# sevagh/umx.cpp

Hardware: AMD Instinct MI355X
Metric: realtime-factor (audio-sec/wall-sec) UMX-L 4-stem, 60 s seg (higher is better)
Workload: dtype f32 (activations as 2 x fp16 planes of the power-of-two-scaled row, integer weights exact in fp16, f32 accumulate on the fp16 matrix cores; fp32-grade: 1.4-2.2x the error of an fp32 evaluation, profiles/r06_v2_accuracy_vs_float64.txt)

## Files before the change

### umx.cpp_amd/__init__.py

```python
import ctypes as C
import os
import subprocess
from pathlib import Path

import numpy as np

from . import ggml

HERE = Path(__file__).resolve().parent
ROOT = HERE.parent
NB, CROP, KX, NOUT, NFFT, HOP = 2049, 1487, 2976, 4098, 4096, 1024
SEGMENT_SAMPLES = 60 * 44100

UMX_OK, ERR_ARG, ERR_HIP, ERR_MODEL, ERR_TIMEOUT, ERR_NODEVICE = 0, 1, 2, 3, 4, 5
DTYPE_F32, DTYPE_U8, DTYPE_U16 = 0, 1, 2
FLAG_NO_WIENER = 0x1
FLAG_SOFTMASK = 0x2
FLAG_LSTM_STEPWISE = 0x10
FLAG_DEBUG_TAPS = 0x20
FLAG_LSTM_FORCE_SAFE = 0x40
FLAG_LSTM_PROFILE = 0x80
FLAG_PRECISE_ACT = 0x1000
FLAG_DEBUG_LSTM_ABORT = 0x2000
FLAG_RESIDUAL = 0x8000
# ... 383 lines not shown
        self._check(self.lib.umx_hip_weight_stems_device(self.h, (C.c_void_p * 4)(*stem_ptrs), n, hip_stream))

    def track_accumulate_device(self, track_ptrs, sum_weight_ptr, weighted_ptrs, offset, n, hip_stream=None):
        self._check(self.lib.umx_hip_track_accumulate_device(self.h, (C.c_void_p * 4)(*track_ptrs), C.c_void_p(sum_weight_ptr),
                                                             (C.c_void_p * 4)(*weighted_ptrs), offset, n, hip_stream))

    def track_normalise_device(self, track_ptrs, sum_weight_ptr, length, hip_stream=None):
        self._check(self.lib.umx_hip_track_normalise_device(self.h, (C.c_void_p * 4)(*track_ptrs), C.c_void_p(sum_weight_ptr), length,
                                                            hip_stream))

    def separate(self, wave, flags=0, shift_offset=None, rate=MODEL_RATE):
        wave = np.asarray(wave, np.float32)
        L = wave.shape[1]
        a = np.ascontiguousarray(wave.T).ravel()
        outs = [np.empty(2 * L, np.float32) for _ in range(4)]
        if rate == MODEL_RATE:
            self.separate_interleaved(a, L, outs, flags, shift_offset)
        else:
            arr = (_fp * 4)(*[o.ctypes.data_as(_fp) for o in outs])
            self._check(self.lib.umx_hip_shift_inference_rate(self.h, a.ctypes.data_as(_fp), L, int(rate),
                                                              -1 if shift_offset is None else shift_offset, arr, flags, None, None))
        return [np.ascontiguousarray(o.reshape(L, 2).T) for o in outs]

    def separate_many(self, waves, flags=0, shift_offsets=None, rates=None):
        nt = len(waves)
        ins = [np.ascontiguousarray(np.asarray(w, np.float32).T).ravel() for w in waves]
        Ls = [np.asarray(w).shape[1] for w in waves]
        outs = [[np.empty(2 * L, np.float32) for _ in range(4)] for L in Ls]
        a = (_fp * nt)(*[x.ctypes.data_as(_fp) for x in ins])
        o = (_fp * (4 * nt))(*[x.ctypes.data_as(_fp) for t4 in outs for x in t4])
        sh = (C.c_int * nt)(*[(-1 if s is None else s) for s in (shift_offsets or [None] * nt)])
        if rates is None:
            self._check(self.lib.umx_hip_separate_tracks(self.h, nt, a, (C.c_int * nt)(*Ls), sh, o, flags, None, None))
        else:
            self._check(self.lib.umx_hip_separate_tracks_rate(self.h, nt, a, (C.c_int * nt)(*Ls), (C.c_int * nt)(*rates), sh, o, flags,
                                                              None, None))
        return [[np.ascontiguousarray(x.reshape(L, 2).T) for x in t4] for t4, L in zip(outs, Ls)]

    def resample_device(self, rate_in, rate_out, in_ptrs, n_in, out_ptrs, n_out, hip_stream=None):
        nb = len(in_ptrs)
        assert len(out_ptrs) == nb
        self._check(self.lib.umx_hip_resample_device(self.h, int(rate_in), int(rate_out), nb, (C.c_void_p * nb)(*in_ptrs), int(n_in),
                                                     (C.c_void_p * nb)(*out_ptrs), int(n_out), hip_stream))

    def separate_interleaved(self, a, L, outs, flags=0, shift_offset=None):
        import time
        arr = (_fp * 4)(*[o.ctypes.data_as(_fp) for o in outs])
        t0 = time.perf_counter()
        if shift_offset is None:
            rc = self.lib.umx_hip_split_inference(self.h, a.ctypes.data_as(_fp), L, arr, flags, None, None)
        else:
            rc = self.lib.umx_hip_shift_inference(self.h, a.ctypes.data_as(_fp), L, shift_offset, arr, flags, None, None)
        dt = time.perf_counter() - t0
        self._check(rc)
        return dt

    def infer_segment(self, wave, flags=0):
        wave = np.asarray(wave, np.float32)
        n = wave.shape[1]
        a = np.ascontiguousarray(wave.T).ravel()
        outs = [np.empty(2 * n, np.float32) for _ in range(4)]
        arr = (_fp * 4)(*[o.ctypes.data_as(_fp) for o in outs])
        self._check(self.lib.umx_hip_infer_segment(self.h, a.ctypes.data_as(_fp), n, arr, flags))
        return [np.ascontiguousarray(o.reshape(n, 2).T) for o in outs]

    def infer_batch(self, waves, flags=0):
        nb = len(waves)
        aud, ns, outs = (C.c_void_p * nb)(), (C.c_int * nb)(), (C.c_void_p * (4 * nb))()
        keep = []
        for i, wv in enumerate(waves):
            if wv is None:
                aud[i], ns[i] = None, 0
                continue
            wv = np.asarray(wv, np.float32)
            a = np.ascontiguousarray(wv.T).ravel()
            o = [np.empty(2 * wv.shape[1], np.float32) for _ in range(4)]
            keep.append((a, o))
            aud[i], ns[i] = a.ctypes.data, wv.shape[1]
            for t in range(4):
                outs[4 * i + t] = o[t].ctypes.data
        self._check(self.lib.umx_hip_infer_batch(self.h, nb, aud, ns, outs, flags))
        res, k = [], 0
        for wv in waves:
            if wv is None:
                res.append(None)
                continue
            n = keep[k][0].size // 2
            res.append([np.ascontiguousarray(o.reshape(n, 2).T) for o in keep[k][1]])
            k += 1
        return res

    def infer_batch_ptrs(self, audio_ptrs, ns, out_ptrs, flags=0, where="device"):
        nb = len(audio_ptrs)
        aud = (C.c_void_p * nb)(*[p or None for p in audio_ptrs])
        n_ = (C.c_int * nb)(*ns)
        outs = (C.c_void_p * (4 * nb))(*[p or None for p in out_ptrs])
        fn = self.lib.umx_hip_infer_batch_device if where == "device" else self.lib.umx_hip_infer_batch_async
        self._check(fn(self.h, nb, aud, n_, outs, flags))

    def infer_segment_device(self, audio_ptr, n, out_ptrs, flags=0):
        arr = (C.c_void_p * 4)(*out_ptrs)
        self._check(self.lib.umx_hip_infer_segment_device(self.h, C.c_void_p(audio_ptr), n, arr, flags))

    def sync(self):
        self._check(self.lib.umx_hip_sync(self.h))

    def last_error(self):
        return self.lib.umx_hip_last_error(self.h).decode()

    def lstm_was_persistent(self):
        return bool(self.lib.umx_hip_lstm_was_persistent(self.h))

    def lstm_mode(self):
        return self.lib.umx_hip_lstm_mode(self.h)

    def lstm_profile(self):
        buf = (C.c_ulonglong * 48)()
        self._check(self.lib.umx_hip_debug_lstm_profile(self.h, buf))
        a = np.array(buf[:], dtype=np.uint64).reshape(3, 2, 8)
        return a

    def gemm_kernel_name(self, mode):
        return self.lib.umx_hip_gemm_kernel_name(self.h, mode).decode()

    def lstm_kernel_name(self):
        return self.lib.umx_hip_lstm_kernel_name(self.h).decode()

    def lstm_placement(self, n=256):
        buf = (C.c_ulonglong * n)()
        self._check(self.lib.umx_hip_debug_lstm_placement(self.h, buf, n))
        a = np.array(buf[:], dtype=np.uint64)
        return [(int(v >> 48) & 15, int(v >> 40) & 255, int(v >> 32) & 255, int(v) & 0xffffffff) for v in a]

    def tap(self, what, target=0):
        n = self.lib.umx_hip_read_tap(self.h, what.encode(), target, None, 0)
        if n < 0:
            raise UmxError(ERR_ARG, f"tap {what!r} unavailable ({n})")
        buf = np.empty(n, np.float32)
        got = self.lib.umx_hip_read_tap(self.h, what.encode(), target, buf.ctypes.data_as(_fp), n)
        if got != n:
            raise UmxError(ERR_HIP, f"tap {what!r} failed ({got})")
        T, H = self.T, self.hidden
        what = what.split("@")[0].split("#")[0]
        if what in ("lstm_l0", "lstm_l1"):
            return buf.reshape(T, H)
        if what == "proj":
            return buf.reshape(T, 4 * H)
        if what in ("spec", "y"):
            return buf.view(np.complex64).reshape(2, T, NB)
        if what in ("mix_mag", "target_mag"):
            return buf.reshape(2, T, NB)
        if what == "x":
            return buf.reshape(T, KX)
        if what in ("fc1", "lstm", "fc2"):
            return buf.reshape(T, H)
        if what == "mask":
            return buf.reshape(T, NOUT)
        return buf

    def stage_times(self, slot=None):
        names = (C.c_char_p * 32)()
        ms = (C.c_float * 32)()
        if slot is None:
            n = self.lib.umx_hip_stage_times(self.h, names, ms, 32)
        else:
            n = self.lib.umx_hip_stage_times_slot(self.h, slot, names, ms, 32)
        return {names[i].decode(): float(ms[i]) for i in range(n)}

    def stage_kernel_times(self, slot=None):
        names = (C.c_char_p * 32)()
        ms = (C.c_float * 32)()
        n = self.lib.umx_hip_stage_times_slot(self.h, 0, names, (C.c_float * 32)(), 32)
        m = self.lib.umx_hip_stage_kernel_times_slot(self.h, -1 if slot is None else slot, ms, 32)
        return {names[i].decode(): float(ms[i]) for i in range(min(n, m))}


HOST_SYMBOLS = ["umx_model_load", "umx_model_free", "umx_model_hidden", "umx_model_n_tensors", "umx_model_views",
                "umx_model_data_bytes", "umx_model_load_progress", "umx_model_dequantize", "umx_wav_load",
                "umx_wav_free", "umx_wav_write_f32", "umx_wav_load_rate", "umx_wav_write_f32_rate", "umx_split_inference", "umx_shift_inference",
                "umx_segment_plan", "umx_transition_weight", "umx_split_inference_carry", "umx_split_inference_targets"]

SEGMENT_FN = C.CFUNCTYPE(C.c_int, C.c_void_p, _fp, C.c_int, C.POINTER(_fp))
RESET_FN = C.CFUNCTYPE(C.c_int, C.c_void_p)
PROGRESS_FN = C.CFUNCTYPE(None, C.c_float, C.c_void_p)


PH_BEGIN_FN = C.CFUNCTYPE(C.c_int, C.c_void_p, _fp, C.c_int)
PH_LAYER_FN = C.CFUNCTYPE(C.c_int, C.c_void_p, C.c_int)
PH_END_FN = C.CFUNCTYPE(C.c_int, C.c_void_p, C.POINTER(_fp))
PH_STATE_FN = C.CFUNCTYPE(C.c_int, C.c_void_p, C.c_int, _fp)
P2P_FN = C.CFUNCTYPE(C.c_int, C.c_void_p, _fp, C.c_size_t, C.c_int)


class PhasedBackend(C.Structure):
    _fields_ = [("begin", PH_BEGIN_FN), ("layer", PH_LAYER_FN), ("end", PH_END_FN), ("get_layer", PH_STATE_FN),
                ("set_layer", PH_STATE_FN), ("layer_floats", C.c_size_t), ("user", C.c_void_p)]


TG_BEGIN_FN = C.CFUNCTYPE(C.c_int, C.c_void_p, _fp, C.c_int, C.c_uint)
TG_STATE_FN = C.CFUNCTYPE(C.c_int, C.c_void_p, C.c_int, C.c_int, _fp)
TG_VOID_FN = C.CFUNCTYPE(C.c_int, C.c_void_p)
TG_MAG_FN = C.CFUNCTYPE(C.c_int, C.c_void_p, C.c_int, _fp)


class TargetBackend(C.Structure):
    _fields_ = [("begin", TG_BEGIN_FN), ("layer", PH_LAYER_FN), ("get_state", TG_STATE_FN), ("set_state", TG_STATE_FN),
                ("masks", TG_VOID_FN), ("get_mag", TG_MAG_FN), ("set_mag", TG_MAG_FN), ("finish", PH_END_FN), ("discard", TG_VOID_FN),
                ("target_layer_floats", C.c_size_t), ("mag_floats", C.c_size_t), ("user", C.c_void_p)]


class P2P(C.Structure):
    _fields_ = [("send", P2P_FN), ("recv", P2P_FN), ("user", C.c_void_p)]


class Backend(C.Structure):
    _fields_ = [("segment", SEGMENT_FN), ("reset", RESET_FN), ("user", C.c_void_p)]


_host = None


def host_lib():
    global _host
    if _host is not None:
        return _host
    path = HERE / "libumx_host.so"
    if not path.exists():
        raise ImportError(f"{path} is missing: run __graft_entry__.build()")
    lib = C.CDLL(str(path))
    lib.umx_model_load.argtypes = [C.c_char_p, C.POINTER(C.c_void_p), C.c_char_p]
    lib.umx_model_free.argtypes = [C.c_void_p]
    lib.umx_model_hidden.argtypes = [C.c_void_p]
    lib.umx_model_n_tensors.argtypes = [C.c_void_p]
    lib.umx_model_views.restype = C.POINTER(TensorView)
    lib.umx_model_views.argtypes = [C.c_void_p]
    lib.umx_model_data_bytes.restype = C.c_size_t
    lib.umx_model_data_bytes.argtypes = [C.c_void_p]
    lib.umx_model_load_progress.restype = C.c_float
    lib.umx_model_load_progress.argtypes = [C.c_void_p]
    lib.umx_model_dequantize.restype = C.c_long
    lib.umx_model_dequantize.argtypes = [C.c_void_p, C.c_int, C.c_char_p, _fp, C.c_size_t]
    lib.umx_wav_load.argtypes = [C.c_char_p, C.POINTER(_fp), C.POINTER(C.c_int), C.POINTER(C.c_int), C.c_char_p]
    lib.umx_wav_free.argtypes = [_fp]
    lib.umx_wav_write_f32.argtypes = [C.c_char_p, _fp, C.c_int, C.c_char_p]
    lib.umx_wav_load_rate.argtypes = [C.c_char_p, C.POINTER(_fp), C.POINTER(C.c_int), C.POINTER(C.c_int), C.POINTER(C.c_int), C.c_char_p]
    lib.umx_wav_write_f32_rate.argtypes = [C.c_char_p, _fp, C.c_int, C.c_int, C.c_char_p]
    lib.umx_split_inference.argtypes = [C.POINTER(Backend), _fp, C.c_int, C.c_int, C.POINTER(_fp), PROGRESS_FN,
                                        C.c_void_p, C.c_char_p]
    lib.umx_shift_inference.argtypes = [C.POINTER(Backend), _fp, C.c_int, C.c_int, C.c_int, C.POINTER(_fp),
                                        PROGRESS_FN, C.c_void_p, C.c_char_p]
    lib.umx_split_inference_carry.argtypes = [C.POINTER(PhasedBackend), C.POINTER(P2P), C.c_int, C.c_int, _fp, C.c_int, C.c_int,
                                              C.POINTER(_fp), C.c_char_p]
    lib.umx_split_inference_targets.argtypes = [C.POINTER(TargetBackend), C.POINTER(P2P), C.c_int, C.c_int, _fp, C.c_int, C.c_int,
                                                C.POINTER(_fp), C.c_char_p]
    lib.umx_segment_plan.argtypes = [C.c_int, C.c_int, C.POINTER(C.c_int), C.POINTER(C.c_int), C.c_int]
    lib.umx_transition_weight.restype = C.c_float
    lib.umx_transition_weight.argtypes = [C.c_int, C.c_int, C.c_int]
    _host = lib
    return lib


class HostError(RuntimeError):
    def __init__(self, code, msg):
        super().__init__(f"umx_host error {code}: {msg}")
        self.code = code


class HostModel:

    def __init__(self, path):
        self.lib = host_lib()
        h = C.c_void_p()
        err = C.create_string_buffer(256)
        rc = self.lib.umx_model_load(str(path).encode(), C.byref(h), err)
        if rc:
            raise HostError(rc, err.value.decode())
        self.h = h
        self.hidden = self.lib.umx_model_hidden(h)
        self.n_tensors = self.lib.umx_model_n_tensors(h)

    def views(self):
        return self.lib.umx_model_views(self.h), self.n_tensors

    def dequantize(self, target, name):
        n = self.lib.umx_model_dequantize(self.h, target, name.encode(), None, 0)
        if n < 0:
            raise KeyError(name)
        a = np.empty(n, np.float32)
        self.lib.umx_model_dequantize(self.h, target, name.encode(), a.ctypes.data_as(_fp), n)
        return a

    def data_bytes(self):
        return self.lib.umx_model_data_bytes(self.h)

    def close(self):
        if getattr(self, "h", None):
            self.lib.umx_model_free(self.h)
            self.h = None

    def __del__(self):
        try:
            self.close()
        except Exception:
            pass


def engine_from_host_model(hm, segment_samples=SEGMENT_SAMPLES, device=0):
# ... 195 lines not shown
```

### umx.cpp_amd/csrc/engine.hip

```cpp
#include "../../include/umx_hip.h"
#include <chrono>
#include <dlfcn.h>

#include <algorithm>
#include <numeric>
#include <cmath>
#include <cstdio>
#include <cstdlib>
#include <cstring>
#include <map>
#include <mutex>
#include <string>
#include <vector>

#include "common.h"
#include "gemm_bf16x3.h"
#include "gemm_planes.h"
#include "gemm_planes_pp.h"
#include "gemm_planes_ps.h"
#include "lstm_kernels.h"
#include "lstm_batch.h"
#include "lstm_batch8.h"
#include "track_kernels.h"
#include "resample.h"
#include "stft_kernels.h"
#include "wiener_kernels.h"
#include "wiener_istft.h"
#include "wiener_em.h"
#include "residual_mask.h"
#include "softmask.h"
#include "gate_debug.h"

using namespace umx;

#define UMX_HIP_CHECK_CTX(ctx_, expr)                                                                                \
    do                                                                                                               \
    {                                                                                                                \
        hipError_t _e = (expr);                                                                                      \
        if (_e != hipSuccess)                                                                                        \
        {                                                                                                            \
            (ctx_)->set_error(std::string(#expr) + ": " + hipGetErrorString(_e));                                    \
            return UMX_ERR_HIP;                                                                                      \
        }                                                                                                            \
    } while (0)

namespace
{
std::string g_create_error = "";

enum { W_FC1 = 0, W_IH0, W_IH1, W_IH2, W_FC2, W_FC3, W_COUNT };
inline int gemm_weight(int mode, int layer) { return mode == G_FC1 ? W_FC1 : mode == G_IH ? W_IH0 + layer : mode == G_FC2 ? W_FC2 : W_FC3; }

struct GemmWeight
{
    const void *p = nullptr;
    int form = 0;
    float s[2] = {1.f, 1.f}, o[2] = {0.f, 0.f};
};

struct TargetBufs
{
    GemmWeight w[W_COUNT];
    float *in_scale = nullptr, *in_mean = nullptr, *bn1[4] = {};
    float *ih_b[3] = {};
    float *bn2[4] = {};
    float *bn3[4] = {}, *out_scale = nullptr, *out_mean = nullptr;
};

struct TargetAct
{
    float *cat = nullptr, *la = nullptr, *lb = nullptr, *P = nullptr, *a2 = nullptr,
          *mag = nullptr;
    unsigned short *xs_p = nullptr, *cat_p = nullptr, *la_p = nullptr, *lb_p = nullptr, *a2_p = nullptr;
    float *rs_xs = nullptr, *rs_catL = nullptr, *rs_catR = nullptr, *rs_la = nullptr, *rs_lb = nullptr, *rs_a2 = nullptr;
    float *rsc_xs = nullptr, *rsc_a2 = nullptr;
};

enum
{
    ST_STFT = 0,
    ST_FC1,
    ST_IH0,
    ST_LSTM0,
    ST_IH1,
    ST_LSTM1,
    ST_IH2,
    ST_LSTM2,
    ST_FC2,
    ST_FC3,
    ST_WIENER,
    ST_ISTFT,
    ST_OLA,
    ST_COUNT
};
enum { SP_XS = 0, SP_CATL, SP_LA, SP_LB, SP_CATR, SP_A2 };
const char *kStageNames[ST_COUNT] = {"stft",  "fc1", "lstm_ih0", "lstm_rec0", "lstm_ih1", "lstm_rec1", "lstm_ih2",
                                     "lstm_rec2", "fc2", "fc3_mask", "wiener",  "istft",    "ola"};

namespace
{
struct RoctxApi
{
    int (*push)(const char *) = nullptr;
    int (*pop)() = nullptr;
    char names[ST_COUNT][40];
    RoctxApi()
    {
        for (int i = 0; i < ST_COUNT; ++i)
            snprintf(names[i], sizeof names[i], "umx:%s", kStageNames[i]);
        const char *want = getenv("UMX_ROCTX");
        const bool force = want && atoi(want) != 0;
        for (const char *lib : {"librocprofiler-sdk-roctx.so", "libroctx64.so"})
            if (void *h = dlopen(lib, force ? (RTLD_NOW | RTLD_LOCAL) : (RTLD_NOW | RTLD_NOLOAD)))
            {
                push = reinterpret_cast<int (*)(const char *)>(dlsym(h, "roctxRangePushA"));
                pop = reinterpret_cast<int (*)()>(dlsym(h, "roctxRangePop"));
                if (push && pop)
                    return;
                push = nullptr;
                pop = nullptr;
            }
    }
};
thread_local bool t_stage_range_open = false;
inline void stage_range(int stage)
{
    static const RoctxApi api;
    if (!api.push)
        return;
    if (t_stage_range_open)
        api.pop();
    t_stage_range_open = stage >= 0 && stage < ST_COUNT;
    if (t_stage_range_open)
        api.push(api.names[stage]);
}
struct StageRangeCloser
{
    ~StageRangeCloser() { stage_range(-1); }
};
}

struct Lane
{
    TargetAct ta[4];
    float2 *spec = nullptr, *y = nullptr, *frames = nullptr;
    float *x = nullptr, *wpart = nullptr, *Rc = nullptr;
    unsigned *maxabs = nullptr;
};

struct Slot
{
    hipStream_t stream = nullptr;
    Lane lane[LSTMB_MAX_TRACKS];
    float *hbuf = nullptr;
    float *wv = nullptr;
    bool lstm_wrote_planes[3] = {false, false, false};
    bool lstm_rows_f32[3] = {true, true, true};
    unsigned *status = nullptr, *lsync = nullptr;
    unsigned long long *lprof = nullptr;
    hipEvent_t ev[ST_COUNT + 1] = {};
    hipEvent_t evk[ST_COUNT] = {};
    bool evk_set[ST_COUNT] = {};
    hipEvent_t rec_done[3] = {};
    hipEvent_t k_done = nullptr;
    hipEvent_t out_free = nullptr;
    bool out_free_valid = false;
    bool have_times = false, last_persistent = false, used = false;
};
}

namespace
{
struct LstmGate
{
    std::mutex m;
    struct Grid
    {
        hipEvent_t done;
        int units;
        hipStream_t stream;
        unsigned long long seq;
    };
    std::vector<Grid> inflight;
    std::vector<hipEvent_t> pool;
    unsigned long long seq = 0;
    int reserved = 0;
    std::vector<int> reservations;
};
LstmGate g_gate[16];

template <class Launch> hipError_t lstm_gate_launch(int device, hipStream_t st, int units, int capacity_units, Launch launch)
{
    LstmGate &g = g_gate[device & 15];
    std::lock_guard<std::mutex> lock(g.m);
    capacity_units -= std::min(g.reserved, capacity_units / 2);
    for (size_t i = 0; i < g.inflight.size();)
        if (hipEventQuery(g.inflight[i].done) == hipSuccess)
        {
            g.pool.push_back(g.inflight[i].done);
            g.inflight.erase(g.inflight.begin() + i);
        }
        else
            ++i;
    (void)hipGetLastError();
    struct PerStream
    {
        hipStream_t stream;
        int units;
        unsigned long long oldest;
        hipEvent_t newest;
    };
    std::vector<PerStream> others;
    for (const LstmGate::Grid &gr : g.inflight)
    {
        if (gr.stream == st)
            continue;
        PerStream *ps = nullptr;
        for (PerStream &o : others)
            if (o.stream == gr.stream)
                ps = &o;
        if (!ps)
        {
            others.push_back({gr.stream, 0, gr.seq, gr.done});
            ps = &others.back();
        }
        ps->units = std::max(ps->units, gr.units);
        ps->newest = gr.done;
    }
    int used = 0;
    for (const PerStream &o : others)
        used += o.units;
    while (used + units > capacity_units && !others.empty())
    {
        size_t k = 0;
        for (size_t i = 1; i < others.size(); ++i)
            if (others[i].oldest < others[k].oldest)
                k = i;
        (void)hipStreamWaitEvent(st, others[k].newest, 0);
        used -= others[k].units;
        others.erase(others.begin() + k);
    }
    hipEvent_t ev = nullptr;
    if (!g.pool.empty())
    {
        ev = g.pool.back();
        g.pool.pop_back();
    }
    else if (hipEventCreateWithFlags(&ev, hipEventDisableTiming) != hipSuccess)
        ev = nullptr;
    const hipError_t e = launch();
    if (ev && e == hipSuccess && hipEventRecord(ev, st) == hipSuccess)
        g.inflight.push_back({ev, units, st, g.seq++});
    else if (ev)
        g.pool.push_back(ev);
    return e;
}
}

template <class K> static const void *kernel_ptr(K *k) { return reinterpret_cast<const void *>(k); }

#ifndef UMX_FUSE_LSTM_PLANES
#define UMX_FUSE_LSTM_PLANES 1
#endif
enum { LSTM_PERSISTENT = 0, LSTM_BATCH, LSTM_BATCH8 };
struct LstmKernel
{
    int family, hl, u8, precise, octets;
    const void *fn;
    size_t lds;
};
#define LSTM_ROW_P(HL, PR) {LSTM_PERSISTENT, HL, -1, PR, 1, kernel_ptr(lstm_persistent_kernel<HL / 8, PR>), 0}
#define LSTM_ROW_B(HL, U8, PR) {LSTM_BATCH, HL, U8, PR, 1, kernel_ptr(lstm_batch_kernel<HL, U8, PR>), lstmb_lds_bytes(LSTMB_GROUP_TRACKS, lstmb_lanes(LSTMB_GROUP_TRACKS).bulk)}
#define LSTM_ROW_8(HL, PR, NO) {LSTM_BATCH8, HL, 1, PR, NO, kernel_ptr(lstm_batch8_kernel<HL, PR, NO>), lstm8_lds_bytes(HL, NO)}
#define LSTM_ROWS_P(HL) LSTM_ROW_P(HL, false), LSTM_ROW_P(HL, true)
#define LSTM_ROWS_B(HL) LSTM_ROW_B(HL, false, false), LSTM_ROW_B(HL, false, true), LSTM_ROW_B(HL, true, false), LSTM_ROW_B(HL, true, true)
#define LSTM_ROWS_8(HL) LSTM_ROW_8(HL, false, 1), LSTM_ROW_8(HL, true, 1), LSTM_ROW_8(HL, false, 2), LSTM_ROW_8(HL, true, 2)
static const LstmKernel kLstmKernels[] = {
    LSTM_ROWS_P(64), LSTM_ROWS_P(128), LSTM_ROWS_P(256), LSTM_ROWS_P(512),
    LSTM_ROWS_B(64), LSTM_ROWS_B(128), LSTM_ROWS_B(256), LSTM_ROWS_B(512),
    LSTM_ROWS_8(256), LSTM_ROWS_8(512),
};
#undef LSTM_ROWS_8
#undef LSTM_ROWS_B
#undef LSTM_ROWS_P
#undef LSTM_ROW_8
#undef LSTM_ROW_B
#undef LSTM_ROW_P
static const LstmKernel *lstm_kernel(int family, int hl, bool u8, bool precise, int octets = 1)
{
    for (const LstmKernel &k : kLstmKernels)
        if (k.family == family && k.hl == hl && (k.u8 < 0 || k.u8 == (int)u8) && k.precise == (int)precise && k.octets == octets)
            return &k;
    return nullptr;
}
static std::string lstm_hidden_sizes(int family)
{
    std::string s;
    int last = 0;
    for (const LstmKernel &k : kLstmKernels)
        if (k.family == family && k.hl != last)
        {
            s += (s.empty() ? "{" : ", ") + std::to_string(2 * k.hl);
            last = k.hl;
        }
    return s + "}";
}

struct GemmKernel
{
    const void *fn = nullptr;
    int lds = 0;
};

template <int MODE> static GemmKernel bx_kernel_m(int bq)
{
    if (bq == BQ_F32)
        return {kernel_ptr(gemm_bf16x3_kernel<MODE, BQ_F32>), BX_LDS_BYTES};
    if constexpr (MODE == G_FC1 || MODE == G_IH)
    {
        if (bq == BQ_U8X)
            return {kernel_ptr(gemm_bf16x3_kernel<MODE, BQ_U8X>), BX_LDS_BYTES};
        if (bq == BQ_U8)
            return {kernel_ptr(gemm_bf16x3_kernel<MODE, BQ_U8>), BX_LDS_BYTES};
    }
    else if (bq == BQ_U16)
        return {kernel_ptr(gemm_bf16x3_kernel<MODE, BQ_U16>), BX_LDS_BYTES};
    return {};
}
static GemmKernel bx_kernel(int mode, int bq)
{
    switch (mode)
    {
    case G_FC1: return bx_kernel_m<G_FC1>(bq);
    case G_IH: return bx_kernel_m<G_IH>(bq);
    case G_FC2: return bx_kernel_m<G_FC2>(bq);
    default: return bx_kernel_m<G_FC3>(bq);
    }
}

enum { GP_128 = 0, GP_256, GP_PP, GP_PS, GP_KINDS };
template <int MODE, int NBP> static GemmKernel gp_kernel_mn(int kind)
{
    switch (kind)
    {
    case GP_128: return {kernel_ptr(gemm_planes_kernel<MODE, NBP, 2, 2>), gp_lds_bytes(2, 2, NBP)};
    case GP_256: return {kernel_ptr(gemm_planes_kernel<MODE, NBP, 4, 4>), gp_lds_bytes(4, 4, NBP)};
    case GP_PP: return {kernel_ptr(gemm_planes_pp_kernel<MODE, NBP>), gp_lds_bytes(4, 4, NBP)};
    default: return {kernel_ptr(gemm_planes_ps_kernel<MODE, NBP>), ps_lds_bytes(NBP)};
    }
}
template <int MODE> static GemmKernel gp_kernel_m(int nbp, int kind)
{
    if constexpr (MODE == G_FC1 || MODE == G_IH)
    {
        if (nbp == 1)
            return gp_kernel_mn<MODE, 1>(kind);
    }
    return nbp == 2 ? gp_kernel_mn<MODE, 2>(kind) : GemmKernel{};
}
static GemmKernel gp_kernel(int mode, int nbp, int kind)
{
    switch (mode)
    {
    case G_FC1: return gp_kernel_m<G_FC1>(nbp, kind);
    case G_IH: return gp_kernel_m<G_IH>(nbp, kind);
    case G_FC2: return gp_kernel_m<G_FC2>(nbp, kind);
    default: return gp_kernel_m<G_FC3>(nbp, kind);
    }
}

struct umx_hip_ctx
{
    int device = 0, H = 0, Hl = 0, S = 0, N = 0, T = 0, Tp = 0, nbatch = 0;
    static constexpr int Mpad = 256;
    std::string err;
    std::vector<void *> allocs;
    TargetBufs tb[4];
    float *whh[3] = {}, *bhh[3] = {};
    float *window = nullptr, *nw = nullptr;
    float2 *tw1 = nullptr, *tw2 = nullptr;
    float *tap_tmp = nullptr;
    float *audio_in = nullptr, *out_dev[4] = {};
    static constexpr int kMaxSlots = 3;
    float *stage_in[kMaxSlots] = {}, *stage_out[kMaxSlots][4 * LSTMB_MAX_TRACKS] = {};
    int ensure_staging();
    hipEvent_t order_ev = nullptr;
    struct DeferredDownload
    {
        bool valid = false;
        int si = 0, nb = 0, n[LSTMB_MAX_TRACKS] = {};
        float *host[4 * LSTMB_MAX_TRACKS] = {};
    };
    int queue_download(const DeferredDownload &d, hipStream_t on);
    hipStream_t copy_stream = nullptr;
    float *state = nullptr, *state_alt = nullptr;
    Slot slot[kMaxSlots];
    int nslots = 2;
    int next_slot() const { return (int)(nseg % nslots); }
    void clear_used()
    {
        for (int si = 0; si < kMaxSlots; ++si)
            slot[si].used = false;
    }
    int B = 1;
    bool lstm_batched = false;
    unsigned tag_epoch = 0;
    unsigned next_tag_base()
    {
        tag_epoch = (tag_epoch + 1) & 0xFFFFF;
        return tag_epoch << 12;
    }
    int cur = 0;
    long long nseg = 0;
    size_t lsync_words = 0;
    bool persistent_ok = true;
    int n_cus = 256;
    struct PendingCall
    {
        int nb;
        const float *audio[LSTMB_MAX_TRACKS];
        int n[LSTMB_MAX_TRACKS];
        float *out[4 * LSTMB_MAX_TRACKS];
        float *host_out[4 * LSTMB_MAX_TRACKS];
        const float *host_audio[LSTMB_MAX_TRACKS];
        unsigned flags;
    };
    static constexpr int kBackupCalls = 8;
    std::vector<PendingCall> pending;
    bool pending_lost = false;
    float *backup = nullptr;
    bool no_recovery = false, recovering = false;
    int recover();
    int lstm_poll_delay = 0;
    int env_gemm_ps = -1;
    int env_gemm_pp = -1;
    const char *gemm_kernel_last[4] = {"none", "none", "none", "none"};
    const char *lstm_kernel_last = "none";
    int lstm_capacity = 0;
    unsigned last_flags = 0;
    hipStream_t stream = nullptr;

    void set_error(const std::string &s) { err = s; }

    template <class T_> int dalloc(T_ **p, size_t count, bool zero = true)
    {
        void *q = nullptr;
        UMX_HIP_CHECK(hipMalloc(&q, std::max<size_t>(count, 1) * sizeof(T_)));
        allocs.push_back(q);
        if (zero)
            UMX_HIP_CHECK(hipMemset(q, 0, std::max<size_t>(count, 1) * sizeof(T_)));
        *p = reinterpret_cast<T_ *>(q);
        return UMX_OK;
    }
    template <class T_> int upload(T_ **p, const std::vector<T_> &h)
    {
        int rc = dalloc(p, h.size(), false);
        if (rc)
            return rc;
        UMX_HIP_CHECK(hipMemcpy(*p, h.data(), h.size() * sizeof(T_), hipMemcpyHostToDevice));
        return UMX_OK;
    }
    int init(int device_, int hidden, int segment_samples, const umx_tensor_view *tensors, int n_tensors,
             unsigned create_flags, int n_tracks);
    size_t weight_bytes = 0;
    bool wiener_fused = true;
    bool gemm_planes = false;
    void launch_split(Lane &ln, int nl, hipStream_t st, int which, const int *active, int nact);
    void launch_gemm_planes(Lane &ln, int nl, hipStream_t st, int mode, int layer, const int *active, int nact, bool dbg);
    void launch_gemm_lanes(Slot &sl, hipStream_t st, int nb, const float *const *audio_dev, int mode, int layer, const int *active,
                           int nact, bool dbg);
    bool u8_dequant = false;
    unsigned char *whh_q[3] = {};
    float whh_s[3][8] = {}, whh_o[3][8] = {};
    int infer_device(const float *audio_dev, int n, float *const out[4], unsigned flags);
    int infer_batch(int nb, const float *const *audio_dev, const int *n, float *const *out , unsigned flags);
    int lstm_batch_capacity = 0;
    bool lstm_batch8_ok = false;
    int lstm8_poll_delay = 0;
    bool env_lstm8_paired = true;
    int env_lstm8_min = 1;
    bool lstm_rowsums = false;
    bool lstm_writes_planes = false;
    size_t state_floats() const { return (size_t)4 * 12 * Hl; }
    int track(const float *audio_host, int length, int shift_offset, float *const out_host[4], unsigned flags,
              void (*progress)(float, void *), void *progress_user);
    int tracks(int nt, const float *const *audio_host, const int *length, const int *shift_offset, float *const *out_host, unsigned flags,
               void (*progress)(float, void *), void *progress_user, const int *rate = nullptr);
    int tracks_once(int nt, const float *const *audio_host, const int *length, const int *shift_offset, float *const *out_host,
                    unsigned flags, void (*progress)(float, void *), void *progress_user, const int *rate);
    std::map<std::pair<int, int>, float *> rs_taps;
    int resample_plan(int rate_in, int rate_out, ResampleGeom &g, const float **taps_dev);
    struct RsStage
    {
        float *in = nullptr, *out[4] = {};
        size_t cap = 0;
    };
    std::vector<RsStage> rs_stage;
    struct TrackBufs
    {
        float *in = nullptr, *out[4] = {}, *sumw = nullptr, *seg[kMaxSlots][4] = {};
        size_t cap = 0;
    };
    std::vector<TrackBufs> trk;
    hipEvent_t trk_acc_ev[kMaxSlots] = {};
    int phase_begin(const float *audio_host, int n, unsigned flags);
    int phase_begin_device(const float *audio_dev, int n, unsigned flags);
    int phase_end_device(float *const out_dev_[4]);
    const float *ph_audio = nullptr;
    int phase_layer(int layer);
    int phase_end(float *const out_host[4]);
    int ph_next = -1;
    int ph_n = 0;
    unsigned ph_flags = 0;
    template <class Args> void fill_lstm_args(Args &a, Slot &sl, int layer, const int *active, int nact);
    int run_lstm_layer(Slot &sl, int layer, const int *active, int nact, bool stepwise, unsigned long long lane_mask);
    int run_lstm_layer_batched(Slot &sl, int layer, const int *active, int nact, bool stepwise, unsigned long long lane_mask);
    int sync_all();
    void launch_gemm(Lane &ln, hipStream_t st, int mode, int layer, const int *active, int nact, bool dbg);
    int stage_front(Slot &sl, hipStream_t st, int nb, const float *const *audio_dev, const int *n, const int *active, int nact);
    WienerStrides lane_strides() const
    {
        WienerStrides ls;
        const size_t nchunk = (size_t)(T + WIENER_CHUNK - 1) / WIENER_CHUNK;
        ls.spec = (size_t)2 * T * NBINS;
        ls.mag = (size_t)2 * T * MAGP;
        ls.part = std::max((size_t)4 * nbatch * NBINS * 9, nchunk * 4 * 5 * NBINS);
        ls.rc = (size_t)4 * NBINS * 4;
        ls.frames = (size_t)4 * T * NFFT;
        ls.y = (size_t)4 * 2 * T * NBINS;
        ls.v = (size_t)4 * T * NBINS;
        return ls;
    }
    static LaneSet lane_set(int nb, const float *const *audio_dev)
    {
        LaneSet l;
        l.count = 0;
        for (int ln = 0; ln < nb; ++ln)
            if (audio_dev[ln])
                l.id[l.count++] = (unsigned char)ln;
        return l;
    }
    int stage_back(Slot &sl, hipStream_t st, int nb, const float *const *audio_dev, float *const *out, const int *n,
                   unsigned flags, const int *active, int nact);
    int stage_masks(Slot &sl, hipStream_t st, int nb, const float *const *audio_dev, unsigned flags, const int *active, int nact);
    int stage_finish(Slot &sl, hipStream_t st, int nb, const float *const *audio_dev, float *const *out, const int *n, unsigned flags,
                     bool zero_skipped);
    int phase_masks();
    int phase_residual();
    int phase_finish_device(float *const out_dev_[4]);
    int check_flags(unsigned flags)
    {
        if (residual_slot_of(flags) != -2)
            return UMX_OK;
        set_error("UMX_FLAG_RESIDUAL needs at least one skipped target (UMX_FLAG_SKIP_TARGET: its slot carries the residual; four targets "
                  "plus a residual would be five sources) and at least one active target");
        return UMX_ERR_ARG;
    }
    void stage_softmask(Slot &sl, hipStream_t st, int nb, const float *const *audio_dev, const int *active, int nact);
    int stage_residual(Slot &sl, hipStream_t st, int nb, const float *const *audio_dev, unsigned flags);
    static void active_list(unsigned flags, int *active, int &nact)
    {
        nact = 0;
        for (int tg = 0; tg < 4; ++tg)
            if (!(flags & UMX_FLAG_SKIP_TARGET(tg)))
                active[nact++] = tg;
    }
};

#include "engine_init.h"
#include "engine_lstm.h"
#include "engine_stages.h"
#include "engine_tracks.h"
#include "engine_phased.h"
#include "engine_cabi.h"
```

### umx.cpp_amd/csrc/engine_cabi.h

```cpp
extern "C"
{

int umx_hip_create(umx_hip_ctx **out, int device, int hidden_size, int segment_samples,
                   const umx_tensor_view *tensors, int n_tensors)
{
    unsigned cf = 0;
    if (const char *e = getenv("UMX_WEIGHTS_RESIDENT"))
        if (std::string(e) == "expanded" || std::string(e) == "f32")
            cf |= UMX_CREATE_DEQUANTISE_AT_LOAD;
    if (const char *e = getenv("UMX_GEMM"))
    {
        if (std::string(e) == "f32")
            cf |= UMX_CREATE_GEMM_F32;
        if (std::string(e) == "bf16x3")
            cf |= UMX_CREATE_GEMM_STAGED;
        if (std::string(e) == "planes")
            cf |= UMX_CREATE_GEMM_PLANES;
    }
    if (const char *e = getenv("UMX_LSTM"))
        if (std::string(e) == "batched")
            cf |= UMX_CREATE_LSTM_BATCHED;
    if (const char *e = getenv("UMX_U8"))
        if (std::string(e) == "dequant")
            cf |= UMX_CREATE_U8_DEQUANT;
// ... 534 lines not shown
        {
            ctx->set_error(hipGetErrorString(e));
            return UMX_ERR_HIP;
        }
        if (st != 0)
        {
            const std::string what = st == 0x80000000u
                                         ? std::string("persistent LSTM kernel: grid barrier timed out (grid not co-resident)")
                                         : "persistent LSTM kernel timed out waiting for a hidden-state granule (code " + std::to_string(st) + ")";
            for (int sj = 0; sj < ctx->nslots; ++sj)
                (void)hipMemset(ctx->slot[sj].status, 0, sizeof(unsigned));
            (void)hipStreamSynchronize(nullptr);
            ctx->persistent_ok = false;
            const size_t ncalls = ctx->pending.size();
            if (!ctx->no_recovery && !ctx->pending_lost && ncalls >= 1 && ncalls <= (size_t)umx_hip_ctx::kBackupCalls)
            {
                const int rc = ctx->recover();
                if (rc == UMX_OK)
                {
                    ctx->set_error("recovered: " + what + "; " + std::to_string(ncalls) + " queued segment call(s) were run again with the "
                                   "per-step LSTM driver (bit-identical), which later calls of this context use as well");
                    return UMX_OK;
                }
            }
            (void)hipMemset(ctx->state, 0, sizeof(float) * ctx->state_floats() * ctx->B);
            (void)hipStreamSynchronize(nullptr);
            ctx->clear_used();
            ctx->pending.clear();
            ctx->pending_lost = false;
            ctx->set_error(what + "; the streaming LSTM state was reset to zero, later segments run the per-step driver");
            return UMX_ERR_TIMEOUT;
        }
    }
    ctx->pending.clear();
    ctx->pending_lost = false;
    return UMX_OK;
}

int umx_hip_infer_batch_async(umx_hip_ctx *ctx, int n_tracks, const float *const *audio_host, const int *n,
                              float *const *out_host, unsigned flags)
{
    if (!ctx || !audio_host || !n || !out_host || n_tracks < 1 || n_tracks > ctx->B)
    {
        if (ctx)
            ctx->set_error("infer: bad arguments");
        return UMX_ERR_ARG;
    }
    if (int rc = ctx->check_flags(flags))
        return rc;
    const int si = ctx->next_slot();
    if (int rc = ctx->ensure_staging())
        return rc;
    Slot &sl = ctx->slot[si];
    hipStream_t st = sl.stream;
    const float *ain[LSTMB_MAX_TRACKS] = {};
    for (int ln = 0; ln < n_tracks; ++ln)
    {
        if (!audio_host[ln])
            continue;
        if (n[ln] < 1 || n[ln] > ctx->N)
        {
            ctx->set_error("infer_segment: need 1 <= n <= segment_samples");
            return UMX_ERR_ARG;
        }
        float *dst = ctx->stage_in[si] + (size_t)2 * ctx->N * ln;
        hipError_t e = hipMemcpyAsync(dst, audio_host[ln], sizeof(float) * 2 * (size_t)n[ln], hipMemcpyHostToDevice, st);
        if (e != hipSuccess)
        {
            ctx->set_error(hipGetErrorString(e));
            return UMX_ERR_HIP;
        }
        ain[ln] = dst;
    }
    if (int rc = ctx->infer_batch(n_tracks, ain, n, ctx->stage_out[si], flags))
        return rc;
    UMX_HIP_CHECK_CTX(ctx, hipEventRecord(sl.k_done, st));
    if (!ctx->pending_lost && !ctx->pending.empty())
    {
        for (int k = 0; k < 4 * n_tracks; ++k)
            ctx->pending.back().host_out[k] = out_host[k];
        for (int ln = 0; ln < n_tracks; ++ln)
            ctx->pending.back().host_audio[ln] = ain[ln] ? audio_host[ln] : nullptr;
    }
    umx_hip_ctx::DeferredDownload d;
    d.valid = true;
    d.si = si;
    d.nb = n_tracks;
    for (int ln = 0; ln < n_tracks; ++ln)
    {
        d.n[ln] = ain[ln] ? n[ln] : 0;
        for (int s = 0; s < 4; ++s)
            d.host[4 * ln + s] = out_host[4 * ln + s];
    }
    return ctx->queue_download(d, ctx->copy_stream);
}

int umx_hip_infer_batch(umx_hip_ctx *ctx, int n_tracks, const float *const *audio_host, const int *n, float *const *out_host,
                        unsigned flags)
{
    if (int rc = umx_hip_infer_batch_async(ctx, n_tracks, audio_host, n, out_host, flags))
        return rc;
    return umx_hip_sync(ctx);
}

int umx_hip_infer_segment_async(umx_hip_ctx *ctx, const float *audio_host, int n, float *const out_host[4], unsigned flags)
{
    if (!ctx || !audio_host || !out_host)
    {
        if (ctx)
            ctx->set_error("infer_segment: bad arguments");
        return UMX_ERR_ARG;
    }
    return umx_hip_infer_batch_async(ctx, 1, &audio_host, &n, out_host, flags);
}

int umx_hip_infer_segment(umx_hip_ctx *ctx, const float *audio_host, int n, float *const out_host[4], unsigned flags)
{
    if (int rc = umx_hip_infer_segment_async(ctx, audio_host, n, out_host, flags))
        return rc;
    return umx_hip_sync(ctx);
}

void *umx_hip_stream_handle(umx_hip_ctx *ctx) { return ctx ? (void *)ctx->slot[ctx->cur].stream : nullptr; }
int umx_hip_nb_frames(const umx_hip_ctx *ctx) { return ctx ? ctx->T : 0; }
int umx_hip_segment_samples(const umx_hip_ctx *ctx) { return ctx ? ctx->N : 0; }
int umx_hip_hidden(const umx_hip_ctx *ctx) { return ctx ? ctx->H : 0; }

long umx_hip_read_tap(umx_hip_ctx *ctx, const char *what, int target, float *dst, size_t cap)
{
    if (!ctx || !what || target < 0 || target > 3)
        return -1;
    std::string w = what;
    const int T = ctx->T, H = ctx->H;
    int which = ctx->cur, lane = 0;
    {
        const size_t hash = w.find('#');
        if (hash != std::string::npos)
        {
            lane = atoi(w.c_str() + hash + 1);
            const size_t at = w.find('@', hash);
            w = w.substr(0, hash) + (at == std::string::npos ? "" : w.substr(at));
            if (lane < 0 || lane >= ctx->B)
                return -1;
        }
    }
    if (w.size() > 2 && w[w.size() - 2] == '@')
    {
        which = w.back() - '0';
        w = w.substr(0, w.size() - 2);
        if (which < 0 || which >= ctx->nslots)
            return -1;
    }
    const Lane &sl = ctx->slot[which].lane[lane];
    const void *src = nullptr;
    size_t nfl = 0, src_ld = 0, rows = 0, cols = 0;
    int computed = 0;
    if (w == "spec") { src = sl.spec; nfl = (size_t)2 * 2 * T * NBINS; }
    else if (w == "mix_mag") { src = sl.spec; computed = 1; nfl = (size_t)2 * T * NBINS; }
    else if (w == "x") { src = sl.x; nfl = (size_t)T * KX; }
    else if (w == "fc1") { src = sl.ta[target].cat; rows = T; cols = H; src_ld = 2 * H; nfl = rows * cols; }
    else if (w == "lstm") { src = sl.ta[target].cat + H; rows = T; cols = H; src_ld = 2 * H; nfl = rows * cols; }
    else if (w == "lstm_l0") { src = sl.ta[target].la; nfl = (size_t)T * H; }
    else if (w == "lstm_l1") { src = sl.ta[target].lb; nfl = (size_t)T * H; }
    else if (w == "proj") { src = sl.ta[target].P; nfl = (size_t)T * 4 * H; }
    else if (w == "fc2") { src = sl.ta[target].a2; nfl = (size_t)T * H; }
    else if (w == "mask") { src = sl.ta[target].mag; computed = 3; nfl = (size_t)T * NOUT; }
    else if (w == "target_mag") { src = sl.ta[target].mag; computed = 2; nfl = (size_t)2 * T * NBINS; }
    else if (w == "y") { src = sl.y + (size_t)target * 2 * T * NBINS; nfl = (size_t)2 * 2 * T * NBINS; }
    else if (w == "max_abs") { src = sl.maxabs; nfl = 1; }
    else return -1;
    if ((w == "lstm" && !ctx->slot[which].lstm_rows_f32[2]) || (w == "lstm_l0" && !ctx->slot[which].lstm_rows_f32[0]) ||
        (w == "lstm_l1" && !ctx->slot[which].lstm_rows_f32[1]))
        return -2;
    if (!src)
        return -2;
    if (!dst)
        return (long)nfl;
    if (cap < nfl)
        return -3;
    if (ctx->sync_all() != UMX_OK)
        return -4;
    if (computed)
    {
        if (!ctx->tap_tmp && ctx->dalloc(&ctx->tap_tmp, (size_t)2 * T * NBINS) != UMX_OK)
            return -4;
        const unsigned blocks = (unsigned)((nfl + 255) / 256);
        if (computed == 1)
            hipLaunchKernelGGL(tap_mix_mag_kernel, dim3(blocks), dim3(256), 0, nullptr, sl.spec, nfl, ctx->tap_tmp);
        else if (computed == 2)
            hipLaunchKernelGGL(tap_target_mag_kernel, dim3(blocks), dim3(256), 0, nullptr, sl.spec, sl.ta[target].mag, nfl, ctx->tap_tmp);
        else
            hipLaunchKernelGGL(tap_mask_kernel, dim3(blocks), dim3(256), 0, nullptr, sl.ta[target].mag, T, ctx->tap_tmp);
        if (hipDeviceSynchronize() != hipSuccess)
            return -4;
        src = ctx->tap_tmp;
    }
    hipError_t e;
    if (rows)
        e = hipMemcpy2D(dst, cols * sizeof(float), src, src_ld * sizeof(float), cols * sizeof(float), rows,
                        hipMemcpyDeviceToHost);
    else
        e = hipMemcpy(dst, src, nfl * sizeof(float), hipMemcpyDeviceToHost);
    if (e != hipSuccess)
    {
        ctx->set_error(hipGetErrorString(e));
        return -4;
    }
    if (w == "max_abs")
    {
        unsigned bits;
        memcpy(&bits, dst, 4);
        float m;
        memcpy(&m, &bits, 4);
        dst[0] = std::max(1.0f, m / WIENER_SCALE);
    }
    return (long)nfl;
}

int umx_hip_stage_times_slot(umx_hip_ctx *ctx, int slot_index, const char **names, float *ms, int cap);
int umx_hip_stage_times(umx_hip_ctx *ctx, const char **names, float *ms, int cap)
{
    return ctx ? umx_hip_stage_times_slot(ctx, ctx->cur, names, ms, cap) : 0;
}

int umx_hip_stage_times_slot(umx_hip_ctx *ctx, int slot_index, const char **names, float *ms, int cap)
{
    if (!ctx || slot_index < 0 || slot_index >= ctx->nslots)
        return 0;
    Slot &sl = ctx->slot[slot_index];
    if (!sl.have_times || ctx->sync_all() != UMX_OK)
        return 0;
    int n = std::min(cap, (int)ST_COUNT);
    for (int i = 0; i < n; ++i)
    {
        float t = 0.f;
        (void)hipEventElapsedTime(&t, sl.ev[i], sl.ev[i + 1]);
        if (names)
            names[i] = kStageNames[i];
        if (ms)
            ms[i] = t;
    }
    return ST_COUNT;
}

int umx_hip_stage_kernel_times_slot(umx_hip_ctx *ctx, int slot_index, float *ms, int cap)
{
    if (ctx && slot_index < 0)
        slot_index = ctx->cur;
    if (!ctx || slot_index >= ctx->nslots)
        return 0;
    Slot &sl = ctx->slot[slot_index];
    if (!sl.have_times || ctx->sync_all() != UMX_OK)
        return 0;
    const int n = std::min(cap, (int)ST_COUNT);
    for (int i = 0; i < n; ++i)
    {
        float t = 0.f;
        (void)hipEventElapsedTime(&t, sl.evk_set[i] ? sl.evk[i] : sl.ev[i], sl.ev[i + 1]);
        if (ms)
            ms[i] = t;
    }
    return ST_COUNT;
}

const char *umx_hip_lstm_kernel_name(const umx_hip_ctx *ctx) { return ctx ? ctx->lstm_kernel_last : "none"; }

const char *umx_hip_gemm_kernel_name(const umx_hip_ctx *ctx, int mode) { return ctx && mode >= 0 && mode < 4 ? ctx->gemm_kernel_last[mode] : "none"; }

int umx_hip_lstm_was_persistent(const umx_hip_ctx *ctx) { return ctx && ctx->slot[ctx->cur].last_persistent ? 1 : 0; }

int umx_hip_lstm_mode(umx_hip_ctx *ctx)
{
    if (!ctx || !ctx->slot[ctx->cur].last_persistent)
        return 0;
    unsigned st[2] = {0, 0};
    const unsigned *src = ctx->slot[ctx->cur].status;
    if (ctx->sync_all() != UMX_OK || hipMemcpy(st, src, sizeof st, hipMemcpyDeviceToHost) != hipSuccess)
        return -1;
    return st[1] ? 2 : 1;
}

int umx_hip_debug_lstm_profile(umx_hip_ctx *ctx, unsigned long long *out48)
{
    if (!ctx || !out48)
        return UMX_ERR_ARG;
    if (ctx->sync_all() != UMX_OK ||
        hipMemcpy(out48, ctx->slot[ctx->cur].lprof, sizeof(unsigned long long) * 48, hipMemcpyDeviceToHost) != hipSuccess)
        return UMX_ERR_HIP;
    return UMX_OK;
}

int umx_hip_debug_lstm_placement(umx_hip_ctx *ctx, unsigned long long *out, int n)
{
    if (!ctx || !out || n < 0 || n > 960 + 64 * 8 * 5)
        return UMX_ERR_ARG;
    if (ctx->sync_all() != UMX_OK ||
        hipMemcpy(out, ctx->slot[ctx->cur].lprof + 64, sizeof(unsigned long long) * n, hipMemcpyDeviceToHost) != hipSuccess)
        return UMX_ERR_HIP;
    return UMX_OK;
}

}
```

### umx.cpp_amd/csrc/engine_init.h

```cpp
namespace
{
bool dequant(const umx_tensor_view &tv, size_t expect, std::vector<float> &out)
{
    size_t nel = 1;
    for (int i = 0; i < tv.n_dims; ++i)
        nel *= (size_t)tv.ne[i];
    if (nel != expect)
        return false;
    out.resize(nel);
    if (tv.dtype == UMX_DTYPE_F32)
        memcpy(out.data(), tv.data, nel * sizeof(float));
    else if (tv.dtype == UMX_DTYPE_U8)
    {
        const uint8_t *q = static_cast<const uint8_t *>(tv.data);
        for (size_t i = 0; i < nel; ++i)
            out[i] = (float)q[i] * tv.scale + tv.offset;
    }
    else if (tv.dtype == UMX_DTYPE_U16)
    {
        const uint16_t *q = static_cast<const uint16_t *>(tv.data);
        for (size_t i = 0; i < nel; ++i)
            out[i] = (float)q[i] * tv.scale + tv.offset;
    }
    else
// ... 290 lines not shown
            if (int rc = upload(&b.bn2[k], v))
                return rc;
            if (!get(tg, std::string("bn3.") + bnn[k], NOUT, v))
                return UMX_ERR_MODEL;
            w.assign(NOUT_PAD, k == 1 ? 1.f : 0.f);
            for (int c = 0; c < 2; ++c)
                memcpy(&w[c * MAGP], &v[c * NBINS], sizeof(float) * NBINS);
            if (int rc = upload(&b.bn3[k], w))
                return rc;
        }
        if (int rc = load_weight(tg, wd[W_FC2], b.w[W_FC2]))
            return rc;
        if (int rc = load_weight(tg, wd[W_FC3], b.w[W_FC3]))
            return rc;
        for (int l = 0; l < 3; ++l)
        {
            if (int rc = load_weight(tg, wd[W_IH0 + l], b.w[W_IH0 + l]))
                return rc;
            std::vector<float> ihb((size_t)2 * G);
            for (int dir = 0; dir < 2; ++dir)
            {
                const std::string sfx = "_l" + std::to_string(l) + (dir ? "_reverse" : "");
                std::vector<float> whhv, bih, bhhv;
                if ((!whh_all_u8 && !get(tg, "lstm.weight_hh" + sfx, (size_t)G * Hl, whhv)) ||
                    !get(tg, "lstm.bias_ih" + sfx, G, bih) || !get(tg, "lstm.bias_hh" + sfx, G, bhhv))
                    return UMX_ERR_MODEL;
                const int chain = tg * 2 + dir;
                const umx_tensor_view *hhv = view(tg, "lstm.weight_hh" + sfx);
                const unsigned char *hhq = whh_all_u8 ? static_cast<const unsigned char *>(hhv->data) : nullptr;
                if (whh_all_u8)
                {
                    whh_s[l][chain] = hhv->scale;
                    whh_o[l][chain] = hhv->offset;
                }
                for (int row = 0; row < G; ++row)
                {
                    const int sl = gate_row[row] / 64, col = gate_row[row] % 64;
                    ihb[(size_t)dir * G + gate_row[row]] = bih[row];
                    bhh_h[l][((size_t)chain * S + sl) * 64 + col] = bhhv[row];
                    for (int k = 0; k < Hl; ++k)
                    {
                        const size_t di = (((size_t)chain * S + sl) * Hl + k) * 64 + col;
                        if (whh_all_u8)
                            whh_qh[l][di] = hhq[(size_t)row * Hl + k];
                        else
                            whh_h[l][di] = whhv[(size_t)row * Hl + k];
                    }
                }
            }
            if (int rc = upload(&b.ih_b[l], ihb))
                return rc;
        }
    }
    for (int l = 0; l < 3; ++l)
    {
        if (whh_all_u8)
        {
            if (int rc = upload(&whh_q[l], whh_qh[l]))
                return rc;
            weight_bytes += whh_qh[l].size();
        }
        else
        {
            if (int rc = upload(&whh[l], whh_h[l]))
                return rc;
            weight_bytes += whh_h[l].size() * sizeof(float);
        }
        if (int rc = upload(&bhh[l], bhh_h[l]))
            return rc;
    }
    {
        std::vector<float> w(NFFT);
        static const float PI = 3.14159265359F;
        const float floatN = (float)(NFFT + 1);
        for (int n = 0; n < NFFT; ++n)
            w[n] = 0.5F * (1.0F - cosf(2.0F * PI * (float)n / (floatN - 1)));
        if (int rc = upload(&window, w))
            return rc;
        const size_t total = (size_t)NFFT + (size_t)HOP * (T - 1);
        std::vector<float> nwh(total, 0.f);
        for (int i = 0; i < T; ++i)
        {
            const size_t s0 = (size_t)i * HOP;
            for (size_t j = s0; j < std::min(total, s0 + NFFT); ++j)
                nwh[j] += w[j - s0] * w[j - s0];
        }
        if (int rc = upload(&nw, nwh))
            return rc;
        std::vector<float2> t1(256), t2(4096);
        for (int r = 0; r < 16; ++r)
            for (int k = 0; k < 16; ++k)
            {
                const double ph = -2.0 * M_PI * (double)(r * k) / 256.0;
                t1[r * 16 + k] = make_float2((float)cos(ph), (float)sin(ph));
            }
        for (int r = 0; r < 16; ++r)
            for (int j = 0; j < 256; ++j)
            {
                const double ph = -2.0 * M_PI * (double)(r * j) / 4096.0;
                t2[r * 256 + j] = make_float2((float)cos(ph), (float)sin(ph));
            }
        if (int rc = upload(&tw1, t1))
            return rc;
        if (int rc = upload(&tw2, t2))
            return rc;
    }
    if (int rc = dalloc(&audio_in, (size_t)2 * N))
        return rc;
    for (int k = 0; k < 4; ++k)
        if (int rc = dalloc(&out_dev[k], (size_t)2 * N))
            return rc;
    if (int rc = dalloc(&state, state_floats() * B))
        return rc;
    if (int rc = dalloc(&state_alt, state_floats() * B))
        return rc;
    if (int rc = dalloc(&backup, (size_t)kBackupCalls * 3 * state_floats() * B))
        return rc;
    lsync_words = LSTM_SYNC_HEADER_WORDS + std::max(granule_count(S) * 2, lstm_batched ? lstmb_granule_words(Hl) * ((B + LSTMB_GROUP_TRACKS - 1) / LSTMB_GROUP_TRACKS) : (size_t)0);
    nslots = 2;
    if (gemm_planes)
    {
        const unsigned long long rows = (unsigned long long)B * Tp + Mpad;
        const unsigned long long planes_bytes = 2ull * rows * (unsigned long long)std::max(KX, 2 * H) * 2ull;
        const unsigned long long mask_bytes = (unsigned long long)B * 2ull * T * MAGP * 4ull;
        if (planes_bytes >= (1ull << 31) || mask_bytes >= (1ull << 32))
        {
            set_error("track lanes x segment length exceed the 32-bit addressing of the plane GEMMs' operands: fewer lanes or a shorter segment");
            return UMX_ERR_ARG;
        }
    }
    for (int si = 0; si < nslots; ++si)
    {
        Slot &sl = slot[si];
        UMX_HIP_CHECK(hipStreamCreateWithFlags(&sl.stream, hipStreamNonBlocking));
        float *x_all = nullptr;
        if (int rc = dalloc(&x_all, ((size_t)B * Tp + Mpad) * KX))
            return rc;
        for (int tg = 0; tg < 4; ++tg)
        {
            float *cat_all = nullptr, *la_all = nullptr, *lb_all = nullptr, *P_all = nullptr, *a2_all = nullptr, *mag_all = nullptr;
            if (int rc = dalloc(&cat_all, ((size_t)B * Tp + Mpad) * 2 * H))
                return rc;
            if (int rc = dalloc(&la_all, ((size_t)B * Tp + Mpad) * H))
                return rc;
            if (int rc = dalloc(&lb_all, ((size_t)B * Tp + Mpad) * H))
                return rc;
            if (int rc = dalloc(&P_all, ((size_t)B * Tp + Mpad) * 4 * H))
                return rc;
            if (int rc = dalloc(&a2_all, ((size_t)B * Tp + Mpad) * H))
                return rc;
            if (int rc = dalloc(&mag_all, (size_t)B * 2 * T * MAGP))
                return rc;
            unsigned short *xs_p = nullptr, *cat_p = nullptr, *la_p = nullptr, *lb_p = nullptr, *a2_p = nullptr;
            float *rs[8] = {};
            if (gemm_planes)
            {
                if (int rc = dalloc(&xs_p, 2 * ((size_t)B * Tp + Mpad) * KX))
                    return rc;
                if (int rc = dalloc(&cat_p, 2 * ((size_t)B * Tp + Mpad) * 2 * H))
                    return rc;
                for (unsigned short **q : {&la_p, &lb_p, &a2_p})
                    if (int rc = dalloc(q, 2 * ((size_t)B * Tp + Mpad) * H))
                        return rc;
                for (int k = 0; k < 8; ++k)
                    if (int rc = dalloc(&rs[k], ((size_t)B * Tp + Mpad) * (k >= 2 && k <= 4 ? 2 : 1)))
                        return rc;
            }
            for (int ln = 0; ln < B; ++ln)
            {
                TargetAct &b = sl.lane[ln].ta[tg];
                b.cat = cat_all + (size_t)ln * Tp * 2 * H;
                b.la = la_all + (size_t)ln * Tp * H;
                b.lb = lb_all + (size_t)ln * Tp * H;
                b.P = P_all + (size_t)ln * Tp * 4 * H;
                b.a2 = a2_all + (size_t)ln * Tp * H;
                b.mag = mag_all + (size_t)ln * 2 * T * MAGP;
                if (gemm_planes)
                {
                    b.xs_p = xs_p + (size_t)ln * Tp * KX;
                    b.cat_p = cat_p + (size_t)ln * Tp * 2 * H;
                    b.la_p = la_p + (size_t)ln * Tp * H;
                    b.lb_p = lb_p + (size_t)ln * Tp * H;
                    b.a2_p = a2_p + (size_t)ln * Tp * H;
                    b.rs_xs = rs[0] + (size_t)ln * Tp;
                    b.rs_catL = rs[1] + (size_t)ln * Tp;
                    b.rs_catR = rs[2] + (size_t)ln * Tp;
                    b.rs_la = rs[3] + (size_t)ln * Tp;
                    b.rs_lb = rs[4] + (size_t)ln * Tp;
                    b.rs_a2 = rs[5] + (size_t)ln * Tp;
                    b.rsc_xs = rs[6] + (size_t)ln * Tp;
                    b.rsc_a2 = rs[7] + (size_t)ln * Tp;
                }
            }
        }
        {
            const WienerStrides ls = lane_strides();
            float2 *spec_all, *y_all, *frames_all;
            float *wpart_all, *Rc_all;
            unsigned *maxabs_all;
            if (int rc = dalloc(&spec_all, (size_t)B * ls.spec))
                return rc;
            if (int rc = dalloc(&y_all, (size_t)B * ls.y))
                return rc;
            if (int rc = dalloc(&frames_all, (size_t)B * ls.frames))
                return rc;
            if (int rc = dalloc(&wpart_all, (size_t)B * ls.part))
                return rc;
            if (int rc = dalloc(&Rc_all, (size_t)B * ls.rc))
                return rc;
            if (int rc = dalloc(&maxabs_all, (size_t)B))
                return rc;
            for (int ln = 0; ln < B; ++ln)
            {
                Lane &L = sl.lane[ln];
                L.x = x_all + (size_t)ln * Tp * KX;
                L.spec = spec_all + (size_t)ln * ls.spec;
                L.y = y_all + (size_t)ln * ls.y;
                L.frames = frames_all + (size_t)ln * ls.frames;
                L.wpart = wpart_all + (size_t)ln * ls.part;
                L.Rc = Rc_all + (size_t)ln * ls.rc;
                L.maxabs = maxabs_all + ln;
            }
        }
        if (int rc = dalloc(&sl.status, 4))
            return rc;
        if (int rc = dalloc(&sl.hbuf, (size_t)2 * 8 * Hl))
            return rc;
        if (int rc = dalloc(&sl.lsync, lsync_words))
            return rc;
        if (int rc = dalloc(&sl.lprof, 1024 + 64 * 8 * 5))
            return rc;
        for (int i = 0; i <= ST_COUNT; ++i)
            UMX_HIP_CHECK(hipEventCreate(&sl.ev[i]));
        for (int i : {ST_FC1, ST_IH0, ST_IH1, ST_IH2, ST_FC2, ST_FC3})
            UMX_HIP_CHECK(hipEventCreate(&sl.evk[i]));
        for (int l = 0; l < 3; ++l)
            UMX_HIP_CHECK(hipEventCreateWithFlags(&sl.rec_done[l], hipEventDisableTiming));
    }
    stream = slot[0].stream;
    {
        int cus = 0;
        UMX_HIP_CHECK(hipDeviceGetAttribute(&cus, hipDeviceAttributeMultiprocessorCount, device));
        n_cus = cus;
        const bool want8 = lstm_batched && B >= env_lstm8_min && !u8_dequant && whh_q[0] && whh_q[1] && whh_q[2];
        const LstmbLanes ll = lstmb_lanes(B);
        constexpr int kNone = 1 << 30;
        int per_cu[3] = {kNone, kNone, kNone};
        for (const LstmKernel &k : kLstmKernels)
        {
            if (k.hl != Hl || (k.family == LSTM_BATCH && !lstm_batched) || (k.family == LSTM_BATCH8 && !want8))
                continue;
            if (k.lds)
                UMX_HIP_CHECK(hipFuncSetAttribute(k.fn, hipFuncAttributeMaxDynamicSharedMemorySize, (int)k.lds));
            int v = 0;
            UMX_HIP_CHECK(hipOccupancyMaxActiveBlocksPerMultiprocessor(&v, k.fn, LSTM_THREADS, k.family == LSTM_BATCH ? lstmb_lds_bytes(ll.nbp, ll.bulk) : k.lds));
            per_cu[k.family] = std::min(per_cu[k.family], v);
        }
        lstm_capacity = per_cu[LSTM_PERSISTENT] == kNone ? 0 : per_cu[LSTM_PERSISTENT] * cus;
        if (lstm_batched)
        {
            if (per_cu[LSTM_BATCH] == kNone)
            {
                set_error("track batching needs hidden_size in " + lstm_hidden_sizes(LSTM_BATCH));
                return UMX_ERR_ARG;
            }
            lstm_batch8_ok = per_cu[LSTM_BATCH8] != kNone && per_cu[LSTM_BATCH8] >= 1 && 8 * 32 <= per_cu[LSTM_BATCH8] * cus;
            lstm_batch_capacity = per_cu[lstm_batch8_ok ? LSTM_BATCH8 : LSTM_BATCH] * cus;
            lstm_rowsums = UMX_FUSE_LSTM_PLANES && gemm_planes && !u8_dequant && whh_q[0] && whh_q[1] && whh_q[2];
            lstm_writes_planes = lstm_rowsums;
        }
    }
    for (const void *fn : {reinterpret_cast<const void *>(wiener_istft_kernel<true>), reinterpret_cast<const void *>(wiener_istft_kernel<false>),
                           reinterpret_cast<const void *>(wiener_istft_v_kernel)})
        UMX_HIP_CHECK(hipFuncSetAttribute(fn, hipFuncAttributeMaxDynamicSharedMemorySize, (int)WI_LDS_BYTES));
    for (int mode = G_FC1; mode <= G_FC3; ++mode)
    {
        std::vector<GemmKernel> ks;
        for (int bq : {BQ_F32, BQ_U8, BQ_U16, BQ_U8X})
            ks.push_back(bx_kernel(mode, bq));
        for (int nbp = 1; nbp <= 2; ++nbp)
            for (int kind = 0; kind < GP_KINDS; ++kind)
                ks.push_back(gp_kernel(mode, nbp, kind));
        for (const GemmKernel &k : ks)
            if (k.fn)
                UMX_HIP_CHECK(hipFuncSetAttribute(k.fn, hipFuncAttributeMaxDynamicSharedMemorySize, k.lds));
    }
    UMX_HIP_CHECK(hipDeviceSynchronize());
    return UMX_OK;
}

int umx_hip_ctx::ensure_staging()
{
    if (stage_in[0])
        return UMX_OK;
    UMX_HIP_CHECK(hipStreamCreateWithFlags(&copy_stream, hipStreamNonBlocking));
    for (int si = 0; si < nslots; ++si)
    {
        for (hipEvent_t *e : {&slot[si].k_done, &slot[si].out_free})
            UMX_HIP_CHECK(hipEventCreateWithFlags(e, hipEventDisableTiming));
        if (int rc = dalloc(&stage_in[si], (size_t)2 * N * B, false))
            return rc;
        for (int k = 0; k < 4 * B; ++k)
            if (int rc = dalloc(&stage_out[si][k], (size_t)2 * N, false))
                return rc;
    }
    return UMX_OK;
}

int umx_hip_ctx::queue_download(const DeferredDownload &d, hipStream_t on)
{
    Slot &src = slot[d.si];
    if (on != src.stream)
        UMX_HIP_CHECK(hipStreamWaitEvent(on, src.k_done, 0));
    for (int ln = 0; ln < d.nb; ++ln)
        if (d.n[ln] > 0)
            for (int s2 = 0; s2 < 4; ++s2)
                UMX_HIP_CHECK(hipMemcpyAsync(d.host[4 * ln + s2], stage_out[d.si][4 * ln + s2], sizeof(float) * 2 * (size_t)d.n[ln],
                                             hipMemcpyDeviceToHost, on));
    UMX_HIP_CHECK(hipEventRecord(src.out_free, on));
    src.out_free_valid = true;
    return UMX_OK;
}

int umx_hip_ctx::sync_all()
{
    for (int si = 0; si < nslots; ++si)
        UMX_HIP_CHECK(hipStreamSynchronize(slot[si].stream));
    if (copy_stream)
        UMX_HIP_CHECK(hipStreamSynchronize(copy_stream));
    for (int si = 0; si < nslots; ++si)
        slot[si].out_free_valid = false;
    return UMX_OK;
}
```

### umx.cpp_amd/csrc/engine_stages.h

```cpp
void umx_hip_ctx::launch_gemm(Lane &sl, hipStream_t st, int mode, int layer, const int *active, int nact, bool dbg)
{
    GemmArgs g;
    memset(&g, 0, sizeof g);
    g.M = Tp;
    g.T = T;
    int bq = BQ_F32;
    for (int i = 0; i < nact; ++i)
    {
        const TargetBufs &b = tb[active[i]];
        const TargetAct &c = sl.ta[active[i]];
        const GemmWeight &w = b.w[gemm_weight(mode, layer)];
        GemmTarget &t = g.t[i];
        switch (mode)
        {
        case G_FC1:
            t.A = sl.x; t.C = c.cat;
            t.e0 = b.bn1[0]; t.e1 = b.bn1[1]; t.e2 = b.bn1[2]; t.e3 = b.bn1[3];
            t.q0 = b.in_scale; t.q1 = b.in_mean;
            g.N = H; g.K = KX; g.lda = KX; g.ldc = 2 * H;
            break;
        case G_IH:
            t.A = layer == 0 ? c.cat : layer == 1 ? c.la : c.lb;
            t.C = c.P; t.e0 = b.ih_b[layer];
            g.N = 4 * H; g.K = H; g.lda = layer == 0 ? 2 * H : H; g.ldc = 4 * H;
            break;
        case G_FC2:
            t.A = c.cat; t.C = c.a2;
            t.e0 = b.bn2[0]; t.e1 = b.bn2[1]; t.e2 = b.bn2[2]; t.e3 = b.bn2[3];
            g.N = H; g.K = 2 * H; g.lda = 2 * H; g.ldc = H;
            break;
        default:
            t.A = c.a2; t.C = c.mag;
            t.e0 = b.bn3[0]; t.e1 = b.bn3[1]; t.e2 = b.bn3[2]; t.e3 = b.bn3[3];
            t.q0 = b.out_scale; t.q1 = b.out_mean;
            g.N = NOUT_PAD; g.K = H; g.lda = H; g.ldc = 0;
            break;
        }
        t.Bq = w.p;
        t.bs[0] = w.s[0]; t.bs[1] = w.s[1];
        t.bo[0] = w.o[0]; t.bo[1] = w.o[1];
        t.bsplit = mode == G_IH ? 2 * H : 0x7fffffff;
        bq = w.form;
    }
    if (bq == BQ_U8 && !u8_dequant)
        bq = BQ_U8X;
    const GemmKernel k = bx_kernel(mode, bq);
    const dim3 grid((unsigned)round_up((g.N / GEMM_BN) * (g.M / GEMM_BM), 8), 1, nact), block(256);
    gemm_kernel_last[mode] = "gemm_bf16x3_kernel";
    void *kargs[] = {&g};
    (void)hipLaunchKernel(k.fn, grid, block, kargs, k.lds, st);
}

void umx_hip_ctx::launch_split(Lane &ln, int nl, hipStream_t st, int which, const int *active, int nact)
{
    SplitArgs a;
    memset(&a, 0, sizeof a);
    a.T = T;
    a.Tp = Tp;
    const size_t rows_all = (size_t)B * Tp + Mpad;
    for (int i = 0; i < nact; ++i)
    {
        const TargetBufs &b = tb[active[i]];
        const TargetAct &c = ln.ta[active[i]];
        switch (which)
        {
        case SP_XS:
            a.src[i] = ln.x; a.dst[i] = c.xs_p; a.rowsum[i] = c.rs_xs; a.rowunscale[i] = c.rsc_xs; a.scale[i] = b.in_scale; a.mean[i] = b.in_mean;
            a.cols = KX; a.ld_src = KX; a.ld_dst = KX; a.col0_dst = 0; a.plane = rows_all * KX;
            break;
        case SP_CATL:
            a.src[i] = c.cat; a.dst[i] = c.cat_p; a.rowsum[i] = c.rs_catL;
            a.cols = H; a.ld_src = 2 * H; a.ld_dst = 2 * H; a.col0_dst = 0; a.plane = rows_all * 2 * H;
            break;
        case SP_CATR:
            a.src[i] = c.cat + H; a.dst[i] = c.cat_p; a.rowsum[i] = lstm_rowsums ? nullptr : c.rs_catR;
            a.cols = H; a.ld_src = 2 * H; a.ld_dst = 2 * H; a.col0_dst = H; a.plane = rows_all * 2 * H;
            break;
        case SP_LA:
            a.src[i] = c.la; a.dst[i] = c.la_p; a.rowsum[i] = lstm_rowsums ? nullptr : c.rs_la;
            a.cols = H; a.ld_src = H; a.ld_dst = H; a.col0_dst = 0; a.plane = rows_all * H;
            break;
        case SP_LB:
            a.src[i] = c.lb; a.dst[i] = c.lb_p; a.rowsum[i] = lstm_rowsums ? nullptr : c.rs_lb;
            a.cols = H; a.ld_src = H; a.ld_dst = H; a.col0_dst = 0; a.plane = rows_all * H;
            break;
        default:
            a.src[i] = c.a2; a.dst[i] = c.a2_p; a.rowsum[i] = c.rs_a2; a.rowunscale[i] = c.rsc_a2;
            a.cols = H; a.ld_src = H; a.ld_dst = H; a.col0_dst = 0; a.plane = rows_all * H;
            break;
        }
    }
    a.rows_valid = nl * Tp;
    const dim3 grid(round_up(nl * Tp, 256) / 4, 1, nact);
    if (which == SP_XS && a.cols <= 3072)
    {
        hipLaunchKernelGGL(split_planes_shared_kernel<6>, dim3(grid.x), dim3(256), 0, st, a, nact);
        return;
    }
    if (a.cols <= 1024)
        hipLaunchKernelGGL(split_planes_kernel<2>, grid, dim3(256), 0, st, a);
    else if (a.cols <= 3072)
        hipLaunchKernelGGL(split_planes_kernel<6>, grid, dim3(256), 0, st, a);
    else
        hipLaunchKernelGGL(split_planes_kernel<8>, grid, dim3(256), 0, st, a);
}

void umx_hip_ctx::launch_gemm_planes(Lane &ln, int nl, hipStream_t st, int mode, int layer, const int *active, int nact, bool dbg)
{
    GemmPArgs g;
    memset(&g, 0, sizeof g);
    g.M = round_up(nl * Tp, 256);
    g.lanes = nl;
    g.T = T;
    g.Tp_lane = Tp;
    g.mag_lane = (size_t)2 * T * MAGP;
    g.a_unscale = 1.0f / (float)(1 << GP_SPLIT_FIXED_EXP);
    const size_t rows_all = (size_t)B * Tp + Mpad;
    int nbp = 2;
    for (int i = 0; i < nact; ++i)
    {
        const TargetBufs &b = tb[active[i]];
        const TargetAct &c = ln.ta[active[i]];
        const GemmWeight &w = b.w[gemm_weight(mode, layer)];
        GemmPTarget &t = g.t[i];
        t.bsplit = 0x7fffffff;
        switch (mode)
        {
        case G_FC1:
            t.A = c.xs_p; t.C = c.cat; t.rs0 = c.rs_xs; t.rsc = c.rsc_xs;
            t.e0 = b.bn1[0]; t.e1 = b.bn1[1]; t.e2 = b.bn1[2]; t.e3 = b.bn1[3];
            g.N = H; g.K = KX; g.lda = KX; g.ldc = 2 * H; g.a_plane = rows_all * KX;
            break;
        case G_IH:
            t.A = layer == 0 ? c.cat_p : layer == 1 ? c.la_p : c.lb_p;
            t.rs0 = layer == 0 ? c.rs_catL : layer == 1 ? c.rs_la : c.rs_lb;
            if (layer > 0 && lstm_rowsums)
                t.rs1 = t.rs0 + rows_all;
            t.C = c.P; t.e0 = b.ih_b[layer];
            t.bsplit = 2 * H;
            g.N = 4 * H; g.K = H; g.lda = layer == 0 ? 2 * H : H; g.ldc = 4 * H;
            g.a_plane = layer == 0 ? rows_all * 2 * H : rows_all * H;
            break;
        case G_FC2:
            t.A = c.cat_p; t.C = c.a2; t.rs0 = c.rs_catL; t.rs1 = c.rs_catR;
            if (lstm_rowsums)
                t.rs2 = c.rs_catR + rows_all;
            t.e0 = b.bn2[0]; t.e1 = b.bn2[1]; t.e2 = b.bn2[2]; t.e3 = b.bn2[3];
            g.N = H; g.K = 2 * H; g.lda = 2 * H; g.ldc = H; g.a_plane = rows_all * 2 * H;
            break;
        default:
            t.A = c.a2_p; t.C = c.mag; t.rs0 = c.rs_a2; t.rsc = c.rsc_a2;
            t.e0 = b.bn3[0]; t.e1 = b.bn3[1]; t.e2 = b.bn3[2]; t.e3 = b.bn3[3];
            t.q0 = b.out_scale; t.q1 = b.out_mean;
            g.N = NOUT_PAD; g.K = H; g.lda = H; g.ldc = 0; g.a_plane = rows_all * H;
            break;
        }
        t.B = static_cast<const unsigned short *>(w.p);
        t.bs[0] = w.s[0]; t.bs[1] = w.s[1];
        t.bo2[0] = w.o[0]; t.bo2[1] = w.o[1];
        nbp = w.form;
    }
    const int blocks_big = (g.N / 256) * (g.M / 256) * nact;
    const bool big = g.N % 256 == 0 && blocks_big >= 224;
    const int bm = big ? 256 : 128;
    const int gemm_pp = env_gemm_pp;
    const bool pp = big && (gemm_pp < 0 || ((gemm_pp >> mode) & 1));
    const int ps_wgs = n_cus / 8 * 8;
    const bool ps = pp && (env_gemm_ps < 0 || ((env_gemm_ps >> mode) & 1)) && g.K / GP_BK >= 6 && ps_wgs >= 8 && blocks_big > ps_wgs && g.Tp_lane >= 256;
    gemm_kernel_last[mode] = ps ? "gemm_planes_ps_kernel" : pp ? "gemm_planes_pp_kernel" : "gemm_planes_kernel";
    const GemmKernel k = gp_kernel(mode, nbp, ps ? GP_PS : pp ? GP_PP : big ? GP_256 : GP_128);
    void *kargs[] = {&g, &nact};
    if (ps)
        (void)hipLaunchKernel(k.fn, dim3(ps_wgs), dim3(512), kargs, k.lds, st);
    else
        (void)hipLaunchKernel(k.fn, dim3((unsigned)round_up((g.N / bm) * (g.M / bm), 8), 1, nact), dim3(pp ? 512 : big ? 1024 : 256), kargs,
                              k.lds, st);
}

void umx_hip_ctx::launch_gemm_lanes(Slot &sl, hipStream_t st, int nb, const float *const *audio_dev, int mode, int layer,
                                    const int *active, int nact, bool dbg)
{
    if (nact <= 0)
        return;
    for (int l0 = 0; l0 < nb;)
    {
        if (!audio_dev[l0])
        {
            ++l0;
            continue;
        }
        int l1 = l0 + 1;
        while (gemm_planes && l1 < nb && audio_dev[l1])
            ++l1;
        if (gemm_planes)
        {
            const int which = mode == G_FC1 ? SP_XS : mode == G_IH ? (layer == 0 ? SP_CATL : layer == 1 ? SP_LA : SP_LB) : mode == G_FC2 ? SP_CATR : SP_A2;
            const int from_layer = which == SP_LA ? 0 : which == SP_LB ? 1 : which == SP_CATR ? 2 : -1;
            if (from_layer < 0 || !sl.lstm_wrote_planes[from_layer])
                launch_split(sl.lane[l0], l1 - l0, st, which, active, nact);
            {
                const int stg = mode == G_FC1 ? ST_FC1 : mode == G_IH ? ST_IH0 + 2 * layer : mode == G_FC2 ? ST_FC2 : ST_FC3;
                sl.evk_set[stg] = sl.evk[stg] && hipEventRecord(sl.evk[stg], st) == hipSuccess;
            }
            launch_gemm_planes(sl.lane[l0], l1 - l0, st, mode, layer, active, nact, dbg);
        }
        else
            launch_gemm(sl.lane[l0], st, mode, layer, active, nact, dbg);
        l0 = l1;
    }
}

int umx_hip_ctx::stage_front(Slot &sl, hipStream_t st, int nb, const float *const *audio_dev, const int *n, const int *active,
                             int nact)
{
    stage_range(ST_STFT);
    for (int i = 0; i < ST_COUNT; ++i)
        sl.evk_set[i] = false;
    UMX_HIP_CHECK(hipEventRecord(sl.ev[ST_STFT], st));
    {
        StftIn in;
        in.lanes = lane_set(nb, audio_dev);
        for (int i = 0; i < in.lanes.count; ++i)
        {
            in.audio[i] = audio_dev[in.lanes.id[i]];
            in.n[i] = n[in.lanes.id[i]];
        }
        Lane &L0 = sl.lane[0];
        UMX_HIP_CHECK(hipMemsetAsync(L0.maxabs, 0, sizeof(unsigned) * B, st));
        hipLaunchKernelGGL(stft_kernel, dim3((T + STFT_RUN - 1) / STFT_RUN, in.lanes.count), dim3(256), 0, st, in, N, T, window, tw1, tw2, L0.spec, lane_strides().spec, L0.x,
                           (size_t)Tp * KX, L0.maxabs);
    }
    stage_range(ST_FC1);
    UMX_HIP_CHECK(hipEventRecord(sl.ev[ST_FC1], st));
    launch_gemm_lanes(sl, st, nb, audio_dev, G_FC1, 0, active, nact, false);
    stage_range(ST_IH0);
    UMX_HIP_CHECK(hipEventRecord(sl.ev[ST_IH0], st));
    launch_gemm_lanes(sl, st, nb, audio_dev, G_IH, 0, active, nact, false);
    return UMX_OK;
}

int umx_hip_ctx::stage_back(Slot &sl, hipStream_t st, int nb, const float *const *audio_dev, float *const *out, const int *n,
                            unsigned flags, const int *active, int nact)
{
    if (int rc = stage_masks(sl, st, nb, audio_dev, flags, active, nact))
        return rc;
    return stage_finish(sl, st, nb, audio_dev, out, n, flags, true);
}

int umx_hip_ctx::stage_masks(Slot &sl, hipStream_t st, int nb, const float *const *audio_dev, unsigned flags, const int *active, int nact)
{
    const bool dbg = flags & UMX_FLAG_DEBUG_TAPS;
    stage_range(ST_FC2);
    UMX_HIP_CHECK(hipEventRecord(sl.ev[ST_FC2], st));
    launch_gemm_lanes(sl, st, nb, audio_dev, G_FC2, 0, active, nact, dbg);
    stage_range(ST_FC3);
    UMX_HIP_CHECK(hipEventRecord(sl.ev[ST_FC3], st));
    launch_gemm_lanes(sl, st, nb, audio_dev, G_FC3, 0, active, nact, dbg);
    if ((flags & UMX_FLAG_SOFTMASK) && nact > 0)
        stage_softmask(sl, st, nb, audio_dev, active, nact);
    UMX_HIP_CHECK(hipGetLastError());
    return UMX_OK;
}

void umx_hip_ctx::stage_softmask(Slot &sl, hipStream_t st, int nb, const float *const *audio_dev, const int *active, int nact)
{
    const LaneSet lanes = lane_set(nb, audio_dev);
    Lane &L0 = sl.lane[0];
    SoftmaskPlanes pl = {};
    for (int i = 0; i < nact; ++i)
        pl.m[i] = L0.ta[active[i]].mag;
    const dim3 grid((2 * T + SM_ROWS - 1) / SM_ROWS, 1, lanes.count), block(256);
    if (nact == 1)
        hipLaunchKernelGGL(softmask_kernel<1>, grid, block, 0, st, pl, L0.spec, T, lanes, lane_strides());
    else if (nact == 2)
        hipLaunchKernelGGL(softmask_kernel<2>, grid, block, 0, st, pl, L0.spec, T, lanes, lane_strides());
    else if (nact == 3)
        hipLaunchKernelGGL(softmask_kernel<3>, grid, block, 0, st, pl, L0.spec, T, lanes, lane_strides());
    else
        hipLaunchKernelGGL(softmask_kernel<4>, grid, block, 0, st, pl, L0.spec, T, lanes, lane_strides());
}

int umx_hip_ctx::stage_residual(Slot &sl, hipStream_t st, int nb, const float *const *audio_dev, unsigned flags)
{
    const int res = residual_slot_of(flags);
    int active[4], nact;
    active_list(flags, active, nact);
    if (res < 0 || nact < 1 || nact > 3)
    {
        set_error("UMX_FLAG_RESIDUAL: no residual slot in these flags");
        return UMX_ERR_ARG;
    }
    const LaneSet lanes = lane_set(nb, audio_dev);
    Lane &L0 = sl.lane[0];
    ResidualSrc src = {};
    for (int i = 0; i < nact; ++i)
        src.m[i] = L0.ta[active[i]].mag;
    const dim3 grid((2 * T + RM_ROWS - 1) / RM_ROWS, 1, lanes.count), block(256);
    if (nact == 1)
        hipLaunchKernelGGL(residual_mask_kernel<1>, grid, block, 0, st, src, L0.ta[res].mag, T, lanes, lane_strides());
    else if (nact == 2)
        hipLaunchKernelGGL(residual_mask_kernel<2>, grid, block, 0, st, src, L0.ta[res].mag, T, lanes, lane_strides());
    else
        hipLaunchKernelGGL(residual_mask_kernel<3>, grid, block, 0, st, src, L0.ta[res].mag, T, lanes, lane_strides());
    return UMX_OK;
}

int umx_hip_ctx::stage_finish(Slot &sl, hipStream_t st, int nb, const float *const *audio_dev, float *const *out, const int *n,
                              unsigned flags, bool zero_skipped)
{
    const bool dbg = flags & UMX_FLAG_DEBUG_TAPS;
    if (zero_skipped)
    {
        const int res = residual_slot_of(flags);
        for (int ln = 0; ln < nb; ++ln)
            if (audio_dev[ln])
                for (int tg = 0; tg < 4; ++tg)
                    if ((flags & UMX_FLAG_SKIP_TARGET(tg)) && tg != res)
                        UMX_HIP_CHECK(hipMemsetAsync(sl.lane[ln].ta[tg].mag, 0, sizeof(float) * 2 * T * MAGP, st));
        if (res >= 0)
            if (int rc = stage_residual(sl, st, nb, audio_dev, flags))
                return rc;
    }
    stage_range(ST_WIENER);
    UMX_HIP_CHECK(hipEventRecord(sl.ev[ST_WIENER], st));
    const int bt = (NBINS + 255) / 256;
    const LaneSet lanes = lane_set(nb, audio_dev);
    const WienerStrides ls = lane_strides();
    Lane &L0 = sl.lane[0];
    WienerMags wm0;
    for (int s = 0; s < 4; ++s)
        wm0.m[s] = L0.ta[s].mag;
    const int nchunk = (T + WIENER_CHUNK - 1) / WIENER_CHUNK;
    const int iters = (flags & UMX_FLAG_NO_WIENER) ? 1 : std::max(1, (int)((flags & UMX_FLAG_WIENER_ITERS_MASK) >> 16));
    if (iters > 1 && !sl.wv)
    {
        if ((unsigned long long)ls.v * sizeof(float) >= (1ull << 31))
        {
            set_error("Wiener EM iterations: the segment's PSD state exceeds the 32-bit addressing of the filter kernel: a shorter segment");
            return UMX_ERR_ARG;
        }
        if (int rc = dalloc(&sl.wv, (size_t)B * ls.v, false))
            return rc;
    }
    if (flags & UMX_FLAG_NO_WIENER)
    {
        if (!wiener_fused)
            for (int i = 0; i < lanes.count; ++i)
            {
                Lane &L = sl.lane[lanes.id[i]];
                WienerMags wm;
                for (int s = 0; s < 4; ++s)
                    wm.m[s] = L.ta[s].mag;
                const size_t nel = (size_t)2 * T * NBINS;
                hipLaunchKernelGGL(mixphase_kernel, dim3((unsigned)((nel + 255) / 256)), dim3(256), 0, st, L.spec, wm, T, L.y);
            }
    }
    else
    {
        hipLaunchKernelGGL(wiener_stats4_kernel<WIENER_STATS_NS>, dim3((NBINS + 63) / 64, nchunk * lanes.count, 4 / WIENER_STATS_NS), dim3(64), 0, st, L0.spec, wm0, T, L0.maxabs, L0.wpart, lanes, ls);
        hipLaunchKernelGGL(wiener_finish4_kernel, dim3(bt, 4, lanes.count), dim3(256), 0, st, L0.wpart, T, L0.Rc, lanes, ls);
        for (int it = 1; it < iters; ++it)
        {
            if (it == 1)
                hipLaunchKernelGGL(wiener_em_step_kernel<true>, dim3((NBINS + 63) / 64, nchunk * lanes.count), dim3(64), 0, st, L0.spec, wm0, sl.wv, T, L0.maxabs, L0.Rc, L0.wpart, lanes, ls);
            else
                hipLaunchKernelGGL(wiener_em_step_kernel<false>, dim3((NBINS + 63) / 64, nchunk * lanes.count), dim3(64), 0, st, L0.spec, wm0, sl.wv, T, L0.maxabs, L0.Rc, L0.wpart, lanes, ls);
            hipLaunchKernelGGL(wiener_finish4_kernel, dim3(bt, 4, lanes.count), dim3(256), 0, st, L0.wpart, T, L0.Rc, lanes, ls);
        }
        if (!wiener_fused)
            for (int i = 0; i < lanes.count; ++i)
            {
                const int ln = lanes.id[i];
                Lane &L = sl.lane[ln];
                WienerMags wm;
                for (int s = 0; s < 4; ++s)
                    wm.m[s] = L.ta[s].mag;
                if (iters > 1)
                    hipLaunchKernelGGL(wiener_apply_kernel<true>, dim3(bt, T), dim3(256), 0, st, L.spec, wm,
                                       reinterpret_cast<const float4 *>(sl.wv + (size_t)ln * ls.v), T, L.maxabs, L.Rc, L.y);
                else
                    hipLaunchKernelGGL(wiener_apply_kernel<false>, dim3(bt, T), dim3(256), 0, st, L.spec, wm, (const float4 *)nullptr, T, L.maxabs, L.Rc, L.y);
            }
    }
    OlaOut oo;
    oo.lanes = lanes;
    int nmax = 1;
    for (int i = 0; i < lanes.count; ++i)
// ... 162 lines not shown
```

### umx.cpp_amd/csrc/gemm_common.h

```cpp
#pragma once
#include <type_traits>
#include "common.h"

namespace umx
{

typedef float floatx16 __attribute__((ext_vector_type(16)));

enum GemmMode
{
    G_FC1 = 0,
    G_IH = 1,
    G_FC2 = 2,
    G_FC3 = 3
};

struct GemmTarget
{
    const float *A;
    const float *B;
    float *C;
    const float *e0, *e1, *e2, *e3;
    const float *q0, *q1;
    const void *Bq;
    float bs[2], bo[2];
    int bsplit;
};

struct GemmArgs
{
    GemmTarget t[4];
    int M, N, K, lda, ldc, T;
    int Tp_lane, lanes;
    size_t mag_lane;
};

#ifndef GEMM_GROUP_M
#define GEMM_GROUP_M 8
#endif
constexpr int GEMM_BM = 128, GEMM_BN = 128;

__device__ __forceinline__ float4 scale_shift(float4 a, float4 sc, float4 mn)
{
    return make_float4(a.x * sc.x + mn.x, a.y * sc.y + mn.y, a.z * sc.z + mn.z, a.w * sc.w + mn.w);
}

__device__ __forceinline__ float tanh_epi(float x)
{
    const float ax = fabsf(x), u = x * x;
    const float e = __builtin_amdgcn_exp2f(ax * -2.88539008177792681f);
    const float big = (1.0f - e) * __builtin_amdgcn_rcpf(1.0f + e);
    float q = fmaf(u, -0.006946978159248829f, 0.021472707390785217f);
    q = fmaf(u, q, -0.05393378809094429f);
    q = fmaf(u, q, 0.1333322674036026f);
    q = fmaf(u, q, -0.3333333134651184f);
    const float small = ax * fmaf(u, q, 1.0f);
    return copysignf(ax < 0.5f ? small : big, x);
}

template <int MODE>
__device__ __forceinline__ void gemm_epilogue(const GemmTarget &tg, const GemmArgs &args, int m0, int n0, int wm, int wn,
                                              int lr, int lh, const floatx16 &acc00, const floatx16 &acc01,
                                              const floatx16 &acc10, const floatx16 &acc11)
{
    int f0 = m0;
    unsigned lo = 0;
    const int tpl = args.Tp_lane ? args.Tp_lane : (1 << 30);
    if (MODE == G_FC3 && args.Tp_lane)
    {
        const int ln = __builtin_amdgcn_readfirstlane(m0 / args.Tp_lane);
        f0 = m0 - ln * args.Tp_lane;
        lo = (unsigned)(ln * args.mag_lane);
    }
    const int m_next = tpl - f0;
    const int mlb = wm * 64 + 4 * lh;
    const int fA = f0 + mlb, fB = mlb - m_next;
    const unsigned dA = ((unsigned)args.mag_lane - (unsigned)args.Tp_lane * MAGP) * 4u;
    const int lanes = args.Tp_lane ? (args.lanes ? args.lanes : args.M / args.Tp_lane) : 1;
    const unsigned mag_bytes = MODE == G_FC3 ? (unsigned)((args.Tp_lane ? (size_t)lanes * args.mag_lane : (size_t)2 * args.T * MAGP) * 4) : 0u;
    const __amdgpu_buffer_rsrc_t rs_mag = __builtin_amdgcn_make_buffer_rsrc(tg.C, 0, mag_bytes, 0x00020000);
#pragma unroll
    for (int ni = 0; ni < 2; ++ni)
    {
        const int n = n0 + wn * 64 + ni * 32 + lr;
        float rm = 0.f, sd = 1.f, rsd = 1.f, gw = 1.f, gb = 0.f, osc = 1.f, omn = 0.f;
        if (MODE == G_IH)
            gb = tg.e0[n];
        else
        {
            rm = tg.e0[n];
            sd = sqrtf(tg.e1[n] + 1e-5f);
            rsd = 1.0f / sd;
            gw = tg.e2[n];
            gb = tg.e3[n];
        }
        unsigned col = (unsigned)n;
        bool col_ok = true;
        if (MODE == G_FC3)
        {
            osc = tg.q0[n];
            omn = tg.q1[n];
            const int c = n >= MAGP ? 1 : 0, bin = n - c * MAGP;
            col = lo + (unsigned)(c * args.T) * MAGP + (unsigned)bin;
            col_ok = bin < NBINS;
        }
        unsigned run = (col + (unsigned)fA * MAGP) * 4u;
        int frow = fB;
#pragma unroll
        for (int mi = 0; mi < 2; ++mi)
#pragma unroll
            for (int rq = 0; rq < 4; ++rq)
            {
                float ys[4];
                unsigned offs[4];
#pragma unroll
                for (int j = 0; j < 4; ++j)
                {
                    const int r = 4 * rq + j;
                    const int ml = wm * 64 + mi * 32 + j + 8 * rq + 4 * lh;
                    float y = mi == 0 ? (ni == 0 ? acc00[r] : acc01[r]) : (ni == 0 ? acc10[r] : acc11[r]);
                    if (MODE == G_IH)
                        tg.C[(size_t)(m0 + ml) * args.ldc + n] = y + gb;
                    else
                    {
                        y = div_by(y - rm, sd, rsd) * gw + gb;
                        if (MODE == G_FC1)
                            tg.C[(size_t)(m0 + ml) * args.ldc + n] = tanh_epi(y);
                        else if (MODE == G_FC2)
                            tg.C[(size_t)(m0 + ml) * args.ldc + n] = fmaxf(y, 0.f);
                        else
                        {
                            const bool second = frow >= 0;
                            const int f = second ? frow : frow + tpl;
                            const bool ok = col_ok && f < args.T;
                            ys[j] = fmaxf(y * osc + omn, 0.f);
                            offs[j] = ok ? run + (second ? dA : 0u) : 0xfffffff0u;
                            run += MAGP * 4;
                            frow += 1;
                        }
                    }
                }
                if (MODE == G_FC3)
                {
#pragma unroll
                    for (int j = 0; j < 4; ++j)
                        __builtin_amdgcn_raw_buffer_store_b32(__float_as_uint(ys[j]), rs_mag, offs[j], 0, 0);
                    run += 4 * MAGP * 4;
                    frow += 4;
                }
                asm volatile("" ::: "memory");
                __builtin_amdgcn_sched_barrier(0);
            }
    }
}

enum GemmBType
{
    BQ_F32 = 0,
    BQ_U8 = 1,
    BQ_U16 = 2,
    BQ_U8X = 3
};

__device__ __forceinline__ float4 deq_u8x4(unsigned p, float sc, float of)
{
    return make_float4((float)(p & 255u) * sc + of, (float)((p >> 8) & 255u) * sc + of,
                       (float)((p >> 16) & 255u) * sc + of, (float)(p >> 24) * sc + of);
}
__device__ __forceinline__ float4 deq_u16x4(uint2 p, float sc, float of)
{
    return make_float4((float)(p.x & 65535u) * sc + of, (float)(p.x >> 16) * sc + of,
                       (float)(p.y & 65535u) * sc + of, (float)(p.y >> 16) * sc + of);
}


}
```

### umx.cpp_amd/csrc/gemm_planes.h

```cpp
#pragma once
#include "gemm_bf16x3.h"
#include <cmath>
#include <cstring>

namespace umx
{

struct GemmPTarget
{
    const unsigned short *A;
    const unsigned short *B;
    float *C;
    const float *e0, *e1, *e2, *e3, *q0, *q1;
    const float *rs0, *rs1, *rs2;
    const float *rsc;
    float bs[2], bo2[2];
    int bsplit;
};

struct GemmPArgs
{
    GemmPTarget t[4];
    int M, N, K, lda, ldc, T;
    size_t a_plane;
    float a_unscale;
    int Tp_lane;
    int lanes;
    size_t mag_lane;
};

constexpr int GP_BK = 32;
constexpr int GP_SPLIT_FIXED_EXP = 14;
__host__ __device__ constexpr int gp_stage_bytes(int WM, int WN, int NBP) { return (2 * 64 * WM + NBP * 64 * WN) * 64; }
__host__ __device__ constexpr int gp_stages(int WM, int WN, int NBP)
{
    return 3 * gp_stage_bytes(WM, WN, NBP) <= (WM * WN >= 16 ? 160 : 80) * 1024 ? 3 : 2;
}
__host__ __device__ constexpr int gp_lds_bytes(int WM, int WN, int NBP) { return gp_stages(WM, WN, NBP) * gp_stage_bytes(WM, WN, NBP); }

__host__ inline unsigned short f16_rne_bits(float f)
{
    unsigned u;
    memcpy(&u, &f, 4);
    const unsigned sign = (u >> 16) & 0x8000u;
    u &= 0x7fffffffu;
    if (u >= 0x7f800000u)
        return (unsigned short)(sign | 0x7c00u | (u > 0x7f800000u ? 0x200u : 0u));
    if (u >= 0x477ff000u)
        return (unsigned short)(sign | 0x7c00u);
    if (u < 0x38800000u)
    {
        if (u < 0x33000000u)
            return (unsigned short)sign;
        float a;
        memcpy(&a, &u, 4);
        const float scaled = a * 16777216.0f;
        const float r = nearbyintf(scaled);
        return (unsigned short)(sign | (unsigned)r);
    }
    const unsigned mant = u & 0x7fffffu, exp = (u >> 23) - 112u;
    unsigned h = (exp << 10) | (mant >> 13);
    const unsigned rem = mant & 0x1fffu;
    if (rem > 0x1000u || (rem == 0x1000u && (h & 1u)))
        ++h;
    return (unsigned short)(sign | h);
}
__host__ inline float f16_bits_to_float(unsigned short h)
{
    const unsigned sign = (unsigned)(h & 0x8000u) << 16, e = (h >> 10) & 31u, m = h & 0x3ffu;
    float v;
    if (e == 0)
        v = ldexpf((float)m, -24);
    else if (e == 31)
        v = m ? NAN : INFINITY;
    else
        v = ldexpf((float)(m | 0x400u), (int)e - 25);
    return sign ? -v : v;
}

struct SplitArgs
{
    const float *src[4];
    unsigned short *dst[4];
    float *rowsum[4];
    float *rowunscale[4];
    const float *scale[4], *mean[4];
    int T, Tp, cols, ld_src, ld_dst, col0_dst;
    int rows_valid;
    size_t plane;
};

typedef _Float16 f16x8 __attribute__((ext_vector_type(8)));

__device__ __forceinline__ void split2_f16(const float (&x)[8], float scale, uint4 &p1, uint4 &p2)
{
    f16x8 h1, h2;
#pragma unroll
    for (int j = 0; j < 8; ++j)
    {
        const float v = x[j] * scale;
        h1[j] = (_Float16)v;
        h2[j] = (_Float16)(v - (float)h1[j]);
    }
    p1 = *reinterpret_cast<uint4 *>(&h1);
    p2 = *reinterpret_cast<uint4 *>(&h2);
}

template <int ITER> __global__ __launch_bounds__(256) void split_planes_kernel(SplitArgs a)
{
    const int tg = blockIdx.z, tid = threadIdx.x, lane = tid & 63;
    const int m = blockIdx.x * 4 + (tid >> 6);
    const float *src = a.src[tg] + (size_t)m * a.ld_src;
    unsigned short *dst = a.dst[tg] + (size_t)m * a.ld_dst + a.col0_dst;
    const float *sc = a.scale[tg], *mn = a.mean[tg];
    const bool adaptive = a.rowunscale[tg] != nullptr;
    const bool live = m < a.rows_valid && m % a.Tp < a.T;
    float xs[ITER][8];
    float sum = 0.f, mx = 0.f;
#pragma unroll
    for (int it = 0; it < ITER; ++it)
    {
        const int k = (it * 64 + lane) * 8;
#pragma unroll
        for (int j = 0; j < 8; ++j)
            xs[it][j] = 0.f;
        if (k < a.cols && live)
        {
            const float4 v0 = stream_load4(src + k), v1 = stream_load4(src + k + 4);
            xs[it][0] = v0.x; xs[it][1] = v0.y; xs[it][2] = v0.z; xs[it][3] = v0.w;
            xs[it][4] = v1.x; xs[it][5] = v1.y; xs[it][6] = v1.z; xs[it][7] = v1.w;
            if (sc)
#pragma unroll
                for (int j = 0; j < 8; ++j)
                    xs[it][j] = xs[it][j] * sc[k + j] + mn[k + j];
        }
        sum += ((xs[it][0] + xs[it][1]) + (xs[it][2] + xs[it][3])) + ((xs[it][4] + xs[it][5]) + (xs[it][6] + xs[it][7]));
#pragma unroll
        for (int j = 0; j < 8; ++j)
            mx = fmaxf(mx, fabsf(xs[it][j]));
    }
#pragma unroll
    for (int off = 32; off >= 1; off >>= 1)
    {
        sum += __shfl_xor(sum, off, 64);
        mx = fmaxf(mx, __shfl_xor(mx, off, 64));
    }
    float scale = (float)(1 << GP_SPLIT_FIXED_EXP), unscale = 1.0f / (float)(1 << GP_SPLIT_FIXED_EXP);
    if (adaptive)
    {
        int e = 0;
        if (mx > 0.f && mx < 3.0e38f)
        {
            int x;
            (void)frexpf(mx, &x);
            e = min(max(GP_SPLIT_FIXED_EXP + 1 - x, -100), 100);
        }
        scale = ldexpf(1.0f, e);
        unscale = ldexpf(1.0f, -e);
    }
    if (lane == 0)
    {
        if (a.rowsum[tg])
            a.rowsum[tg][m] = sum;
        if (adaptive)
            a.rowunscale[tg][m] = unscale;
    }
#pragma unroll
    for (int it = 0; it < ITER; ++it)
    {
        const int k = (it * 64 + lane) * 8;
        if (k < a.cols)
        {
            uint4 p1, p2;
            split2_f16(xs[it], scale, p1, p2);
            stream_store4u(reinterpret_cast<uint4 *>(dst + k), p1);
            stream_store4u(reinterpret_cast<uint4 *>(dst + a.plane + k), p2);
        }
    }
}

template <int ITER> __global__ __launch_bounds__(256) void split_planes_shared_kernel(SplitArgs a, int ntargets)
{
// ... 147 lines not shown
#define GP_MFMA(A, B, C) C = __builtin_amdgcn_mfma_f32_32x32x16_f16(A, B, C, 0, 0, 0);
#define GP_TERM(PA, PB, KK)                                                                                          \
    {                                                                                                                \
        const int co = (((KK)*2 + lh) ^ sw) * 16;                                                                    \
        const f16x8 b0 = GP_LD(bo + fragB + (PB)*B_PL + co);                                                         \
        const f16x8 b1 = GP_LD(bo + fragB + (PB)*B_PL + 32 * 64 + co);                                               \
        _Pragma("unroll") for (int mi = 0; mi < MI; ++mi)                                                            \
        {                                                                                                            \
            const f16x8 am = GP_LD(bo + fragA + (PA)*A_PL + mi * 32 * 64 + co);                                      \
            GP_MFMA(am, b0, acc[mi][0]) GP_MFMA(am, b1, acc[mi][1])                                                  \
        }                                                                                                            \
    }
#define GP_COMPUTE(buf)                                                                                              \
    {                                                                                                                \
        const int bo = (buf)*BUF_BYTES;                                                                              \
        _Pragma("unroll") for (int kk = 0; kk < 2; ++kk)                                                             \
        {                                                                                                            \
            if (NBP == 1)                                                                                            \
            {                                                                                                        \
                GP_TERM(1, 0, kk) GP_TERM(0, 0, kk)                                                                  \
            }                                                                                                        \
            else  \
            {                                                                                                        \
                GP_TERM(1, 0, kk) GP_TERM(0, 1, kk) GP_TERM(0, 0, kk)                                                \
            }                                                                                                        \
        }                                                                                                            \
    }

#define GP_WAIT(n) __builtin_amdgcn_s_waitcnt(0x0f70 | (n))
    const int nk = K / GP_BK;
    GP_DMA(0, 0)
    if (STAGES == 3 && nk > 1)
    {
        GP_DMA(1, GP_BK)
        GP_WAIT(DMA_PER_WAVE);
    }
    else
        GP_WAIT(0);
    __syncthreads();
#ifndef GP_EXPERIMENT_NO_DMA
#define GP_EXPERIMENT_NO_DMA 0
#endif
#ifndef GP_EXPERIMENT_NO_MFMA
#define GP_EXPERIMENT_NO_MFMA 0
#endif
#ifndef GP_PROFILE
#define GP_PROFILE 0
#endif
    [[maybe_unused]] long long pf[4] = {0, 0, 0, 0};
    if (STAGES == 3)
    {
        int cur = 0;
        for (int kt = 0; kt < nk - 2; ++kt)
        {
            const int nxt = cur == 0 ? 2 : cur - 1;
            [[maybe_unused]] long long c0 = 0, c1 = 0, c2 = 0, c3 = 0;
            if (GP_PROFILE)
                c0 = clock64();
            if (!GP_EXPERIMENT_NO_DMA)
                GP_DMA(nxt, (kt + 2) * GP_BK)
            if (GP_PROFILE)
                c1 = clock64();
            if (!GP_EXPERIMENT_NO_MFMA)
                GP_COMPUTE(cur)
            if (GP_PROFILE)
                c2 = clock64();
            GP_WAIT(DMA_PER_WAVE);
            if (GP_PROFILE)
                c3 = clock64();
            __syncthreads();
            if (GP_PROFILE)
            {
                const long long c4 = clock64();
                pf[0] += c1 - c0;
                pf[1] += c2 - c1;
                pf[2] += c3 - c2;
                pf[3] += c4 - c3;
            }
            cur = cur == 2 ? 0 : cur + 1;
        }
        if (GP_PROFILE && blockIdx.x == 64 && blockIdx.z == 0 && (tid == 0 || tid == 64 * 7))
            printf("# gemm_planes<%d,%d> wave %d trips %d: cycles per trip  dma-issue %lld  fragments+mfma %lld  wait-dma %lld  barrier %lld\n", MODE, NBP,
                   wave, nk - 2, pf[0] / (nk - 2), pf[1] / (nk - 2), pf[2] / (nk - 2), pf[3] / (nk - 2));
        if (nk > 1)
        {
            GP_COMPUTE(cur)
            GP_WAIT(0);
            __syncthreads();
            cur = cur == 2 ? 0 : cur + 1;
        }
        GP_COMPUTE(cur)
    }
    else
    {
        for (int kt = 0; kt < nk - 1; ++kt)
        {
            const int cur = kt & 1;
            if (!GP_EXPERIMENT_NO_DMA)
                GP_DMA(cur ^ 1, (kt + 1) * GP_BK)
            if (!GP_EXPERIMENT_NO_MFMA)
                GP_COMPUTE(cur)
            GP_WAIT(0);
            __syncthreads();
        }
        GP_COMPUTE((nk - 1) & 1)
    }
#undef GP_WAIT
#undef GP_DMA
#undef GP_LD
#undef GP_MFMA
#undef GP_TERM
#undef GP_COMPUTE
    {
        const int sel = n0 >= tg.bsplit ? 1 : 0;
        const float bsc = tg.bs[sel], o2 = tg.bo2[sel];
        float *const fx = reinterpret_cast<float *>(gp_smem);
        __syncthreads();
        for (int i = tid; i < BM; i += 64 * NW)
        {
            const int m = m0 + i;
            fx[i] = bsc * (tg.rsc ? tg.rsc[m] : args.a_unscale);
            fx[BM + i] = o2 * (tg.rs2 ? (tg.rs0[m] + tg.rs1[m]) + tg.rs2[m] : tg.rs1 ? tg.rs0[m] + tg.rs1[m] : tg.rs0[m]);
        }
        __syncthreads();
#pragma unroll
        for (int mi = 0; mi < MI; ++mi)
#pragma unroll
            for (int rq = 0; rq < 4; ++rq)
            {
                const int ml = wm * 32 * MI + mi * 32 + 8 * rq + 4 * lh;
                const float4 mu = *reinterpret_cast<const float4 *>(fx + ml), ad = *reinterpret_cast<const float4 *>(fx + BM + ml);
                const float mus[4] = {mu.x, mu.y, mu.z, mu.w}, ads[4] = {ad.x, ad.y, ad.z, ad.w};
#pragma unroll
                for (int j = 0; j < 4; ++j)
                {
                    const int r = 4 * rq + j;
                    acc[mi][0][r] = mus[j] * acc[mi][0][r] + ads[j];
                    acc[mi][1][r] = mus[j] * acc[mi][1][r] + ads[j];
                }
                asm volatile("" ::: "memory");
            }
    }
    GemmTarget et;
    et.C = tg.C;
    et.e0 = tg.e0; et.e1 = tg.e1; et.e2 = tg.e2; et.e3 = tg.e3;
    et.q0 = tg.q0; et.q1 = tg.q1;
    GemmArgs ea;
    ea.M = args.M;
    ea.ldc = args.ldc;
    ea.T = args.T;
    ea.Tp_lane = args.Tp_lane;
    ea.lanes = args.lanes;
    ea.mag_lane = args.mag_lane;
#pragma unroll
    for (int half = 0; half < MI / 2; ++half)
        gemm_epilogue<MODE>(et, ea, m0 + wm * 32 * MI + half * 64, n0, 0, wn, lr, lh, acc[2 * half][0], acc[2 * half][1], acc[2 * half + 1][0],
                            acc[2 * half + 1][1]);
}

}
```

### umx.cpp_amd/csrc/gemm_planes_pp.h

```cpp
#pragma once
#include "gemm_planes.h"

#ifndef PP_DMA_BOTH
#define PP_DMA_BOTH 1
#endif

namespace umx
{

template <int MODE, int NBP> __global__ __launch_bounds__(512, 1) void gemm_planes_pp_kernel(GemmPArgs args)
{
    extern __shared__ __attribute__((aligned(16))) unsigned char gp_smem[];
    constexpr int MI = 4, BM = 256, BN = 256;
    constexpr int A_PL = BM * 64, B_PL = BN * 64;
    constexpr int BUF_BYTES = 2 * A_PL + NBP * B_PL, STAGES = gp_stages(4, 4, NBP);
    constexpr int PH = 1, KKP = 2 / PH;
    static_assert(NBP == 1 || NBP == 2, "weight planes: 1 (u8) or 2 (u16, fp32)");
    const GemmPTarget tg = args.t[blockIdx.z];
    const int tid = threadIdx.x, lane = tid & 63, wave = __builtin_amdgcn_readfirstlane(tid >> 6);
    const int grp = wave >> 2, ws = wave & 3;
    const int wm = grp, wn = ws, lr = lane & 31, lh = lane >> 5;
    int tile_m, tile_n;
    {
        const int gx = args.N / BN, gy = args.M / BM, total = gx * gy;
// ... 72 lines not shown
    {                                                                                                                \
        PP_MFMA(fa[PA][mi][kl], fb[PB][0][kl], acc[mi][0]) PP_MFMA(fa[PA][mi][kl], fb[PB][1][kl], acc[mi][1])        \
    }
#define PP_MMA()                                                                                                     \
    _Pragma("unroll") for (int kl = 0; kl < KKP; ++kl)                                                               \
    {                                                                                                                \
        if (NBP == 1)                                                                                                \
        {                                                                                                            \
            PP_TERM(1, 0, kl) PP_TERM(0, 0, kl)                                                                      \
        }                                                                                                            \
        else                                                                                                         \
        {                                                                                                            \
            PP_TERM(1, 0, kl) PP_TERM(0, NBP - 1, kl) PP_TERM(0, 0, kl)                                              \
        }                                                                                                            \
    }
#define PP_WAIT_VM(n) __builtin_amdgcn_s_waitcnt(0x0f70 | ((n) & 15) | (((n) >> 4) << 14))
#define PP_WAIT_LDS() __builtin_amdgcn_s_waitcnt(0xc07f)
#define PP_BARRIER()                                                                                                 \
    {                                                                                                                \
        __builtin_amdgcn_sched_barrier(0);                                                                           \
        __builtin_amdgcn_s_barrier();                                                                                \
        __builtin_amdgcn_sched_barrier(0);                                                                           \
    }

#ifndef PP_EXPERIMENT
#define PP_EXPERIMENT 0
#endif
#ifndef PP_PROFILE
#define PP_PROFILE 0
#endif
    [[maybe_unused]] long long pq[6] = {0, 0, 0, 0, 0, 0};
    if (PP_PROFILE)
        pq[0] = clock64();
    const int nk = K / GP_BK;
    if (grp == 0 || BOTH)
    {
        PP_DMA(0, 0)
        if (STAGES == 3 && nk > 1)
        {
            PP_DMA(1, GP_BK)
            PP_WAIT_VM(DMA_PER_WAVE);
        }
        else
            PP_WAIT_VM(0);
    }
    PP_BARRIER()
    if (PP_PROFILE)
        pq[1] = clock64();
    if (grp == 1)
        PP_BARRIER()
    int cur = 0;
    for (int kt = 0; kt < nk; ++kt)
    {
        const int nxt = STAGES == 3 ? (cur == 0 ? 2 : cur - 1) : cur ^ 1;
#pragma unroll
        for (int ph = 0; ph < PH; ++ph)
        {
            if (!(PP_EXPERIMENT & 1) && ph == 0 && (grp == 0 || BOTH) && kt + STAGES - 1 < nk)
                PP_DMA(nxt, (kt + STAGES - 1) * GP_BK)
            if (!(PP_EXPERIMENT & 4) || kt == 0)
                PP_LOAD(cur, ph)
            PP_WAIT_LDS();
            if (BOTH && grp == 1 && kt + 1 < nk)
            {
                if (kt + 2 < nk)
                    PP_WAIT_VM(DMA_PER_WAVE);
                else
                    PP_WAIT_VM(0);
            }
            PP_BARRIER()
            __builtin_amdgcn_s_setprio(1);
            if (!(PP_EXPERIMENT & 2) || kt == 0)
                PP_MMA()
            __builtin_amdgcn_s_setprio(0);
            if (ph == PH - 1 && grp == 0 && kt + 1 < nk)
            {
                if (STAGES == 3 && kt + 2 < nk)
                    PP_WAIT_VM(DMA_PER_WAVE);
                else
                    PP_WAIT_VM(0);
            }
            PP_BARRIER()
        }
        cur = cur + 1 == STAGES ? 0 : cur + 1;
    }
    if (grp == 0)
        PP_BARRIER()
    if (PP_PROFILE)
        pq[2] = clock64();
#undef PP_DMA
#undef PP_LD
#undef PP_LOAD
#undef PP_MFMA
#undef PP_TERM
#undef PP_MMA
#undef PP_WAIT_VM
#undef PP_WAIT_LDS
#undef PP_BARRIER
    {
        const int sel = n0 >= tg.bsplit ? 1 : 0;
        const float bsc = tg.bs[sel], o2 = tg.bo2[sel];
        float *const fx = reinterpret_cast<float *>(gp_smem);
        __syncthreads();
        for (int i = tid; i < BM; i += 512)
        {
            const int m = m0 + i;
            fx[i] = bsc * (tg.rsc ? tg.rsc[m] : args.a_unscale);
            fx[BM + i] = o2 * (tg.rs2 ? (tg.rs0[m] + tg.rs1[m]) + tg.rs2[m] : tg.rs1 ? tg.rs0[m] + tg.rs1[m] : tg.rs0[m]);
        }
        __syncthreads();
#pragma unroll
        for (int mi = 0; mi < MI; ++mi)
#pragma unroll
            for (int rq = 0; rq < 4; ++rq)
            {
                const int ml = wm * 32 * MI + mi * 32 + 8 * rq + 4 * lh;
                const float4 mu = *reinterpret_cast<const float4 *>(fx + ml), ad = *reinterpret_cast<const float4 *>(fx + BM + ml);
                const float mus[4] = {mu.x, mu.y, mu.z, mu.w}, ads[4] = {ad.x, ad.y, ad.z, ad.w};
#pragma unroll
                for (int j = 0; j < 4; ++j)
                {
                    const int r = 4 * rq + j;
                    acc[mi][0][r] = mus[j] * acc[mi][0][r] + ads[j];
                    acc[mi][1][r] = mus[j] * acc[mi][1][r] + ads[j];
                }
                asm volatile("" ::: "memory");
            }
    }
    if (PP_PROFILE)
        pq[3] = clock64();
    GemmTarget et;
    et.C = tg.C;
    et.e0 = tg.e0; et.e1 = tg.e1; et.e2 = tg.e2; et.e3 = tg.e3;
    et.q0 = tg.q0; et.q1 = tg.q1;
    GemmArgs ea;
    ea.M = args.M;
    ea.ldc = args.ldc;
    ea.T = args.T;
    ea.Tp_lane = args.Tp_lane;
    ea.lanes = args.lanes;
    ea.mag_lane = args.mag_lane;
    if (PP_EXPERIMENT & 8)
    {
        float s = 0.f;
#pragma unroll
        for (int mi = 0; mi < MI; ++mi)
#pragma unroll
            for (int r = 0; r < 16; ++r)
                s += acc[mi][0][r] + acc[mi][1][r];
        if (s == 12345.678f)
            tg.C[tid] = s;
        return;
    }
#pragma unroll
    for (int half = 0; half < MI / 2; ++half)
        gemm_epilogue<MODE>(et, ea, m0 + wm * 32 * MI + half * 64, n0, 0, wn, lr, lh, acc[2 * half][0], acc[2 * half][1], acc[2 * half + 1][0],
                            acc[2 * half + 1][1]);
    if (PP_PROFILE)
    {
        pq[4] = clock64();
        __builtin_amdgcn_s_waitcnt(0x0f70);
        pq[5] = clock64();
        if ((blockIdx.x == 264 || blockIdx.x == 2000) && blockIdx.z == 1 && (tid == 0 || tid == 64 * 4))
            printf("# pp<%d,%d> wg %d wave %d trips %d: cycles  first-tile-wait %lld  main-loop %lld (%lld per trip)  fix-up %lld  epilogue-issue %lld  store-drain %lld  total %lld\n",
                   MODE, NBP, (int)blockIdx.x, wave, nk, pq[1] - pq[0], pq[2] - pq[1], (pq[2] - pq[1]) / nk, pq[3] - pq[2], pq[4] - pq[3], pq[5] - pq[4], pq[5] - pq[0]);
    }
}

}
```

### umx.cpp_amd/csrc/gemm_planes_ps.h

```cpp
#pragma once
#include "gemm_planes_pp.h"

namespace umx
{

typedef float floatx4 __attribute__((ext_vector_type(4)));
typedef unsigned int v4u32 __attribute__((ext_vector_type(4)));
constexpr int PS_TAB_ROWS = 4, PS_TAB_COLS = 8;
__host__ __device__ constexpr int ps_lds_bytes(int NBP) { return gp_lds_bytes(4, 4, NBP) + (PS_TAB_ROWS + PS_TAB_COLS) * 256 * 4; }
constexpr unsigned PS_DROP = 0x40000000u;
#ifndef PS_STORE_AUX
#define PS_STORE_AUX 2
#endif
#ifndef PS_PREWAIT
#define PS_PREWAIT 1
#endif
#ifndef PS_A_AUX
#define PS_A_AUX 0
#endif
#ifndef PS_B_AUX
#define PS_B_AUX 0
#endif
#ifndef PS_PROFILE
#define PS_PROFILE 0
#endif

template <int MODE, int NBP> __global__ __launch_bounds__(512, 1) void gemm_planes_ps_kernel(GemmPArgs args, int ntg)
{
    extern __shared__ __attribute__((aligned(16))) unsigned char gp_smem[];
    constexpr int MI = 4, BM = 256, BN = 256, KKP = 2;
    constexpr int A_PL = BM * 64, B_PL = BN * 64;
    constexpr int BUF_BYTES = 2 * A_PL + NBP * B_PL, STAGES = gp_stages(4, 4, NBP);
    static_assert(NBP == 1 || NBP == 2, "weight planes: 1 (u8) or 2 (u16, fp32)");
    float *const rowtab = reinterpret_cast<float *>(gp_smem + STAGES * BUF_BYTES);
    float *const coltab = rowtab + PS_TAB_ROWS * 256;
    const int tid = threadIdx.x, lane = tid & 63, wave = __builtin_amdgcn_readfirstlane(tid >> 6);
    const int grp = wave >> 2, ws = wave & 3;
    const int wm = grp, wn = ws, lr = lane & 31, lh = lane >> 5;
    const int K = args.K, lda = args.lda, nk = K / GP_BK;

    const int gx = args.N / BN, gy = args.M / BM, total = gx * gy, total_all = total * ntg;
    const int wpx = (int)gridDim.x >> 3, chunk = (total_all + 7) >> 3;
    const int v_begin = (int)(blockIdx.x & 7) * chunk + (int)(blockIdx.x >> 3), v_end = min(((int)(blockIdx.x & 7) + 1) * chunk, total_all);
    if (v_begin >= v_end)
        return;
    const int ntiles = (v_end - v_begin + wpx - 1) / wpx, ntrips = ntiles * nk;
#define PS_DECODE(v_, TGI, M0, N0, LN0, F0)                                                                          \
    {                                                                                                                \
        const int tg_ = (v_) / total, vt_ = (v_) - tg_ * total;                                                      \
        const int per_group_ = GEMM_GROUP_M * gx, group_ = vt_ / per_group_, first_m_ = group_ * GEMM_GROUP_M;       \
        const int gsize_ = min(gy - first_m_, GEMM_GROUP_M), in_group_ = vt_ - group_ * per_group_;                  \
        const int q_ = in_group_ / gsize_;                                                                           \
        TGI = tg_;                                                                                                   \
        M0 = (first_m_ + in_group_ - q_ * gsize_) * BM;                                                              \
        N0 = q_ * BN;                                                                                                \
        if (MODE == G_FC3)                                                                                           \
        {                                                                                                            \
            LN0 = M0 / args.Tp_lane;                                                                                 \
            F0 = M0 - LN0 * args.Tp_lane;                                                                            \
        }                                                                                                            \
    }

    typedef __attribute__((address_space(3))) void *lds_ptr;
    const int st_chunk = (lane & 3) ^ ((lane >> 4) & 3);
    const int voffA = ((lane >> 2) * lda) * 2 + st_chunk * 16, voffB = ((lane >> 2) * K) * 2 + st_chunk * 16;
    const unsigned lds0 = (unsigned)(size_t)(lds_ptr)gp_smem;
    constexpr bool BOTH = PP_DMA_BOTH && STAGES == 3;
    constexpr int DEAL = BOTH ? 8 : 4, PER = 16 / DEAL;
    constexpr int A_GROUPS = 2 * (BM / 16), B_GROUPS = NBP * (BN / 16), NA = A_GROUPS / DEAL, NB = B_GROUPS / DEAL, DMA_PER_WAVE = NA + NB;
    static_assert(DMA_PER_WAVE <= 16 && A_GROUPS % DEAL == 0 && B_GROUPS % DEAL == 0 && BM == 256 && BN == 256, "vmcnt bookkeeping below");
    const int w8 = (BOTH ? 4 * grp : 0) + ws;
    const bool issuer = grp == 0 || BOTH;
    const unsigned lds_w = lds0 + (unsigned)w8 * 1024u;
    int a_it[NA], b_it[NB];
#pragma unroll
    for (int it = 0; it < NA; ++it)
        a_it[it] = (int)((long)(it / PER) * (long)args.a_plane * 2) + (it % PER) * DEAL * 32 * lda;
#pragma unroll
    for (int it = 0; it < NB; ++it)
        b_it[it] = (int)((long)(it / PER) * (long)args.N * K * 2) + (it % PER) * DEAL * 32 * K;
    int d_tile = 0, d_k = 0, koff = 0, a_tile, b_tile, n_tgi, n_m0, n_n0, n_ln0 = 0, n_f0 = 0;
    PS_DECODE(v_begin, n_tgi, n_m0, n_n0, n_ln0, n_f0)
    __amdgpu_buffer_rsrc_t rsA = __builtin_amdgcn_make_buffer_rsrc(const_cast<unsigned short *>(args.t[n_tgi].A), 0, 0x7fffffff, 0x00020000);
    __amdgpu_buffer_rsrc_t rsB = __builtin_amdgcn_make_buffer_rsrc(const_cast<unsigned short *>(args.t[n_tgi].B), 0, 0x7fffffff, 0x00020000);
    a_tile = (int)((long)(n_m0 + 16 * w8) * lda * 2);
    b_tile = (int)((long)(n_n0 + 16 * w8) * K * 2);
    int c_tgi = n_tgi, c_m0 = n_m0, c_n0 = n_n0, c_ln0 = n_ln0, c_f0 = n_f0;
#define PS_DMA_ISSUE(buf)                                                                                            \
    {                                                                                                                \
        const unsigned lb_ = lds_w + (unsigned)((buf)*BUF_BYTES);                                                    \
        const int ao_ = a_tile + koff, bo_ = b_tile + koff;                                                          \
        _Pragma("unroll") for (int it = 0; it < NA; ++it)                                                            \
        {                                                                                                            \
            const int so_ = ao_ + a_it[it];                                                                          \
            __builtin_amdgcn_raw_ptr_buffer_load_lds(rsA, (lds_ptr)(size_t)(lb_ + (it / PER) * A_PL + (it % PER) * DEAL * 1024), 16, voffA, so_, 0, PS_A_AUX); \
        }                                                                                                            \
        _Pragma("unroll") for (int it = 0; it < NB; ++it)                                                            \
        {                                                                                                            \
            const int so_ = bo_ + b_it[it];                                                                          \
            __builtin_amdgcn_raw_ptr_buffer_load_lds(rsB, (lds_ptr)(size_t)(lb_ + 2 * A_PL + (it / PER) * B_PL + (it % PER) * DEAL * 1024), 16, voffB, so_, 0, PS_B_AUX); \
        }                                                                                                            \
    }
#define PS_DMA_ADVANCE()                                                                                             \
    {                                                                                                                \
        koff += 2 * GP_BK;                                                                                           \
        if (++d_k == nk)                                                                                             \
        {                                                                                                            \
            d_k = 0;                                                                                                 \
            koff = 0;                                                                                                \
            if (++d_tile < ntiles)                                                                                   \
            {                                                                                                        \
                PS_DECODE(v_begin + d_tile * wpx, n_tgi, n_m0, n_n0, n_ln0, n_f0)                                    \
                rsA = __builtin_amdgcn_make_buffer_rsrc(const_cast<unsigned short *>(args.t[n_tgi].A), 0, 0x7fffffff, 0x00020000); \
                rsB = __builtin_amdgcn_make_buffer_rsrc(const_cast<unsigned short *>(args.t[n_tgi].B), 0, 0x7fffffff, 0x00020000); \
                a_tile = (int)((long)(n_m0 + 16 * w8) * lda * 2);                                                    \
                b_tile = (int)((long)(n_n0 + 16 * w8) * K * 2);                                                      \
            }                                                                                                        \
        }                                                                                                            \
    }

    floatx16 acc[MI][2];
    const floatx16 zero16 = {0.f, 0.f, 0.f, 0.f, 0.f, 0.f, 0.f, 0.f, 0.f, 0.f, 0.f, 0.f, 0.f, 0.f, 0.f, 0.f};
    const int sw = (lr >> 2) & 3;
    const int fragA = (wm * 32 * MI + lr) * 64, fragB = 2 * A_PL + (wn * 64 + lr) * 64;
    f16x8 fa[2][MI][KKP], fb[NBP][2][KKP];
#define PS_LD(off) (*reinterpret_cast<const f16x8 *>(gp_smem + (off)))
#define PS_LOAD_KL(buf, kl)                                                                                          \
    {                                                                                                                \
        const int bo = (buf)*BUF_BYTES;                                                                              \
        const int co = (((kl)*2 + lh) ^ sw) * 16;                                                                    \
        _Pragma("unroll") for (int p = 0; p < NBP; ++p)                                                              \
        {                                                                                                            \
            fb[p][0][kl] = PS_LD(bo + fragB + p * B_PL + co);                                                        \
            fb[p][1][kl] = PS_LD(bo + fragB + p * B_PL + 32 * 64 + co);                                              \
        }                                                                                                            \
        _Pragma("unroll") for (int p = 1; p >= 0; --p)                                                               \
            _Pragma("unroll") for (int mi = 0; mi < MI; ++mi)                                                        \
                fa[p][mi][kl] = PS_LD(bo + fragA + p * A_PL + mi * 32 * 64 + co);                                    \
    }
#define PS_MFMA(A, B, C) __builtin_amdgcn_mfma_f32_32x32x16_f16(A, B, C, 0, 0, 0)
#define PS_BAND(mi, kl, ZERO)                                                                                        \
    {                                                                                                                \
        acc[mi][0] = PS_MFMA(fa[1][mi][kl], fb[0][0][kl], (ZERO) ? zero16 : acc[mi][0]);                             \
        acc[mi][1] = PS_MFMA(fa[1][mi][kl], fb[0][1][kl], (ZERO) ? zero16 : acc[mi][1]);                             \
        if (NBP == 2)                                                                                                \
        {                                                                                                            \
            acc[mi][0] = PS_MFMA(fa[0][mi][kl], fb[NBP - 1][0][kl], acc[mi][0]);                                     \
            acc[mi][1] = PS_MFMA(fa[0][mi][kl], fb[NBP - 1][1][kl], acc[mi][1]);                                     \
        }                                                                                                            \
        acc[mi][0] = PS_MFMA(fa[0][mi][kl], fb[0][0][kl], acc[mi][0]);                                               \
        acc[mi][1] = PS_MFMA(fa[0][mi][kl], fb[0][1][kl], acc[mi][1]);                                               \
    }
#define PS_TERM(PA, PB, kl)                                                                                          \
    _Pragma("unroll") for (int mi = 0; mi < MI; ++mi)                                                                \
    {                                                                                                                \
        acc[mi][0] = PS_MFMA(fa[PA][mi][kl], fb[PB][0][kl], acc[mi][0]);                                             \
        acc[mi][1] = PS_MFMA(fa[PA][mi][kl], fb[PB][1][kl], acc[mi][1]);                                             \
    }
#define PS_STEP(kl)                                                                                                  \
    {                                                                                                                \
        PS_TERM(1, 0, kl)                                                                                            \
        if (NBP == 2)                                                                                                \
            PS_TERM(0, NBP - 1, kl)                                                                                  \
        PS_TERM(0, 0, kl)                                                                                            \
    }
#define PS_WAIT_VM(n) __builtin_amdgcn_s_waitcnt(0x0f70 | ((n) & 15) | (((n) >> 4) << 14))
#define PS_WAIT_LDS() __builtin_amdgcn_s_waitcnt(0xc07f)
#define PS_BARRIER()                                                                                                 \
    {                                                                                                                \
        __builtin_amdgcn_sched_barrier(0);                                                                           \
        __builtin_amdgcn_s_barrier();                                                                                \
        __builtin_amdgcn_sched_barrier(0);                                                                           \
    }

    int e_m0 = 0, e_n0 = 0, e_tgi = 0, e_ln0 = 0, e_f0 = 0;
    __amdgpu_buffer_rsrc_t rsC = __builtin_amdgcn_make_buffer_rsrc(args.t[0].C, 0, 0, 0x00020000);
    const unsigned ldc4 = (unsigned)args.ldc * 4u;
    const float4 *const row4 = reinterpret_cast<const float4 *>(rowtab);
    const uint4 *const row4u = reinterpret_cast<const uint4 *>(rowtab);
    float cv[2][7];
    unsigned cvo[2];
    float4 nx_mu, nx_ad;
    uint4 nx_ro;
    int e_row = 0;
#define PS_EPI_ROWS(g_)                                                                                              \
    {                                                                                                                \
        nx_mu = row4[e_row + 2 * (g_)];                                                                              \
        nx_ad = row4[64 + e_row + 2 * (g_)];                                                                         \
        nx_ro = row4u[128 + e_row + 2 * (g_)];                                                                       \
    }
#define PS_EPI_SETUP()                                                                                               \
    {                                                                                                                \
        int el_ = lane;                                                                                              \
        asm volatile("" : "+v"(el_));                                                                                \
        e_row = wm * 32 + (el_ >> 5);                                                                                \
        _Pragma("unroll") for (int ni = 0; ni < 2; ++ni)                                                             \
        {                                                                                                            \
            const int cl_ = wn * 64 + ni * 32 + (el_ & 31);                                                          \
            cvo[ni] = (unsigned)cl_ * 4u;                                                                            \
            cv[ni][4] = coltab[4 * 256 + cl_];                                                                       \
            if (MODE != G_IH)                                                                                        \
            {                                                                                                        \
                cv[ni][0] = coltab[cl_];                                                                             \
                cv[ni][1] = coltab[256 + cl_];                                                                       \
                cv[ni][2] = coltab[2 * 256 + cl_];                                                                   \
                cv[ni][3] = coltab[3 * 256 + cl_];                                                                   \
            }                                                                                                        \
            if (MODE == G_FC3)                                                                                       \
            {                                                                                                        \
                cv[ni][5] = coltab[5 * 256 + cl_];                                                                   \
                cv[ni][6] = coltab[6 * 256 + cl_];                                                                   \
                cvo[ni] = reinterpret_cast<const unsigned *>(coltab)[7 * 256 + cl_];                                 \
            }                                                                                                        \
        }                                                                                                            \
        PS_EPI_ROWS(0)                                                                                               \
        if (MODE == G_FC3)                                                                                           \
        {                                                                                                            \
            const size_t lane_b_ = args.mag_lane * 4, all_b_ = (size_t)(args.lanes ? args.lanes : args.M / args.Tp_lane) * lane_b_; \
            const size_t lo_ = (size_t)e_ln0 * lane_b_, rest_ = all_b_ > lo_ ? all_b_ - lo_ : 0;                      \
            rsC = __builtin_amdgcn_make_buffer_rsrc(reinterpret_cast<unsigned char *>(args.t[e_tgi].C) + lo_, 0,     \
                                                    (int)(rest_ < 2 * lane_b_ ? rest_ : 2 * lane_b_), 0x00020000);   \
        }                                                                                                            \
        else                                                                                                         \
            rsC = __builtin_amdgcn_make_buffer_rsrc(args.t[e_tgi].C + ((size_t)e_m0 * args.ldc + e_n0), 0, 0x7fffffff, 0x00020000); \
    }
#define PS_EPI_BAND(mi)                                                                                              \
    _Pragma("unroll") for (int rq = 0; rq < 4; ++rq)                                                                 \
    {                                                                                                                \
        const float mus_[4] = {nx_mu.x, nx_mu.y, nx_mu.z, nx_mu.w}, ads_[4] = {nx_ad.x, nx_ad.y, nx_ad.z, nx_ad.w};  \
        const unsigned ro_[4] = {nx_ro.x, nx_ro.y, nx_ro.z, nx_ro.w};                                                \
        if ((mi)*4 + rq + 1 < 16)                                                                                    \
            PS_EPI_ROWS((mi)*4 + rq + 1)                                                                             \
        float ys_[2][4];                                                                                             \
        unsigned os_[2][4];                                                                                          \
        _Pragma("unroll") for (int ni = 0; ni < 2; ++ni)                                                             \
            _Pragma("unroll") for (int j = 0; j < 4; ++j)                                                            \
            {                                                                                                        \
                float y = mus_[j] * acc[mi][ni][4 * rq + j] + ads_[j];                                               \
                if (MODE == G_IH)                                                                                    \
                    y = y + cv[ni][4];                                          \
                else                                                                                                 \
                {                                                                                                    \
                    y = div_by(y - cv[ni][0], cv[ni][1], cv[ni][2]) * cv[ni][3] + cv[ni][4];  \
                    if (MODE == G_FC1)                                                                               \
                        y = tanh_epi(y);                                                                             \
                    else if (MODE == G_FC2)                                                                          \
                        y = fmaxf(y, 0.f);                                                                           \
                    else                                                                                             \
                        y = fmaxf(y * cv[ni][5] + cv[ni][6], 0.f);              \
                }                                                                                                    \
                ys_[ni][j] = y;                                                                                      \
                os_[ni][j] = ro_[j] + cvo[ni];                                                                       \
            }                                                                                                        \
        __builtin_amdgcn_sched_barrier(0);  \
        _Pragma("unroll") for (int ni = 0; ni < 2; ++ni)                                                             \
            _Pragma("unroll") for (int j = 0; j < 4; ++j)                                                            \
                __builtin_amdgcn_raw_buffer_store_b32(__float_as_uint(ys_[ni][j]), rsC, os_[ni][j], 0, PS_STORE_AUX);   \
        __builtin_amdgcn_sched_barrier(0);                                                                           \
    }

    const unsigned lds_row = lds0 + STAGES * BUF_BYTES, lds_col = lds_row + PS_TAB_ROWS * 1024;
#define PS_TAB_PIECE(PTR, LDSOFF, FIRST_ELEM)                                                                        \
    {                                                                                                                \
        if (PTR)                                                                                                     \
            __builtin_amdgcn_raw_ptr_buffer_load_lds(__builtin_amdgcn_make_buffer_rsrc(const_cast<float *>(PTR), 0, 0x7fffffff, 0x00020000), \
                                                     (lds_ptr)(size_t)((LDSOFF) + ws * 256), 4, lane * 4, ((FIRST_ELEM) + ws * 64) * 4, 0, 0); \
    }
#define PS_TAB_RAW()                                                                                                 \
    {                                                                                                                \
        const GemmPTarget &tg_ = args.t[c_tgi];                                                                      \
        if (!BOTH || grp == 0)                                                                                       \
        {                                                                                                            \
            PS_TAB_PIECE(tg_.rsc, lds_row, c_m0)                                                                     \
            PS_TAB_PIECE(tg_.rs0, lds_row + 1024, c_m0)                                                              \
            PS_TAB_PIECE(tg_.rs1, lds_row + 2048, c_m0)                                                              \
            PS_TAB_PIECE(tg_.rs2, lds_row + 3072, c_m0)                                                              \
        }                                                                                                            \
        if (!BOTH || grp == 1)                                                                                       \
        {                                                                                                            \
            if (MODE == G_IH)                                                                                        \
                PS_TAB_PIECE(tg_.e0, lds_col + 4 * 1024, c_n0)                                                       \
            else                                                                                                     \
            {                                                                                                        \
                PS_TAB_PIECE(tg_.e0, lds_col, c_n0)                                                                  \
                PS_TAB_PIECE(tg_.e1, lds_col + 1024, c_n0)                                                           \
                PS_TAB_PIECE(tg_.e2, lds_col + 3 * 1024, c_n0)                                                       \
                PS_TAB_PIECE(tg_.e3, lds_col + 4 * 1024, c_n0)                                                       \
            }                                                                                                        \
            if (MODE == G_FC3)                                                                                       \
            {                                                                                                        \
                PS_TAB_PIECE(tg_.q0, lds_col + 5 * 1024, c_n0)                                                       \
                PS_TAB_PIECE(tg_.q1, lds_col + 6 * 1024, c_n0)                                                       \
            }                                                                                                        \
        }                                                                                                            \
    }
#define PS_TAB_FINISH()                                                                                              \
    {                                                                                                                \
        if (grp == 0)                                                                                                \
        {                                                                                                            \
            const GemmPTarget &tg_ = args.t[e_tgi];                                                                  \
            const int sel_ = e_n0 >= tg_.bsplit ? 1 : 0;                                                             \
            const float rsc_ = tg_.rsc ? rowtab[tid] : args.a_unscale, r0_ = rowtab[256 + tid];                      \
            const float r1_ = tg_.rs1 ? rowtab[512 + tid] : 0.f, r2_ = tg_.rs2 ? rowtab[768 + tid] : 0.f;            \
            unsigned off_ = (unsigned)tid * ldc4;                        \
            if (MODE == G_FC3)                                                                                       \
            {                                                                                                        \
                                                      \
                const int f1_ = e_f0 + tid, second_ = f1_ >= args.Tp_lane ? 1 : 0, f_ = f1_ - second_ * args.Tp_lane; \
                off_ = f_ < args.T ? ((unsigned)second_ * (unsigned)args.mag_lane + (unsigned)f_ * MAGP) * 4u : PS_DROP; \
            }                                                                                                        \
            rowtab[tid] = tg_.bs[sel_] * rsc_;                            \
            rowtab[256 + tid] = tg_.bo2[sel_] * (tg_.rs2 ? (r0_ + r1_) + r2_ : tg_.rs1 ? r0_ + r1_ : r0_);           \
            reinterpret_cast<unsigned *>(rowtab)[512 + tid] = off_;                                                  \
            if (MODE != G_IH)                                                                                        \
            {                                                                                                        \
                const float sd_ = sqrtf(coltab[256 + tid] + 1e-5f);                         \
                coltab[256 + tid] = sd_;                                                                             \
                coltab[2 * 256 + tid] = 1.0f / sd_;                                                                  \
            }                                                                                                        \
            if (MODE == G_FC3)                                                                                       \
            {                                                                                                        \
                          \
                const int n_ = e_n0 + tid, ch_ = n_ >= MAGP ? 1 : 0, bin_ = n_ - ch_ * MAGP;                         \
                reinterpret_cast<unsigned *>(coltab)[7 * 256 + tid] = bin_ < NBINS ? ((unsigned)(ch_ * args.T) * MAGP + (unsigned)bin_) * 4u : PS_DROP; \
            }                                                                                                        \
        }                                                                                                            \
    }

    int cur = 0, u = 0;
#define PS_M(FIRST, LATE, YOUNG1, TAB, FINISH, SPLIT)                                                                       \
    {                                                                                                                \
        const int nxt_ = STAGES == 3 ? (cur == 0 ? 2 : cur - 1) : cur ^ 1;  \
        const bool more_ = u + STAGES - 1 < ntrips, late_ = (LATE) && grp == 0;                                      \
        if ((TAB) && issuer)                                                                                         \
            PS_TAB_RAW()                                                                                             \
        if (more_ && !late_)                                                                                         \
        {                                                                                                            \
            if (issuer)                                                                                              \
                PS_DMA_ISSUE(nxt_)                                                                                   \
            PS_DMA_ADVANCE()                                                                                         \
        }                                                                                                            \
        PS_LOAD_KL(cur, 0)                                                                                           \
        if (!(FIRST))                                                                                                \
            PS_LOAD_KL(cur, 1)                                                                                       \
        if (FINISH)                                                                                                  \
            PS_TAB_FINISH()                                                                                          \
        PS_WAIT_LDS();                                                                                               \
        if (BOTH && grp == 1 && u + 1 < ntrips)                                                                      \
        {                                                                                                            \
             \
            if (YOUNG1)                                                                                              \
            {                                                                                                        \
                if (!PS_PREWAIT)                                                                                     \
                    PS_WAIT_VM(63);                                                                                  \
            }                                                                                                        \
            else if (u + 2 < ntrips)                                                                                 \
                PS_WAIT_VM(DMA_PER_WAVE);                                                                            \
            else                                                                                                     \
                PS_WAIT_VM(0);                                                                                       \
        }                                                                                                            \
        if (!(SPLIT) || grp == 0)              \
            PS_BARRIER()                                                                                             \
        if (more_ && late_)                                                                                          \
        {                                                                                                            \
            PS_DMA_ISSUE(nxt_)                                                                                       \
            PS_DMA_ADVANCE()                                                                                         \
        }                                                                                                            \
    }
#define PS_C_END(YOUNG0)                                                                                             \
    {                                                                                                                \
        if (grp == 0 && u + 1 < ntrips)                                                                              \
        {                                                                                                            \
            if (YOUNG0)                                                                                              \
            {                                                                                                        \
                if (!PS_PREWAIT)                                                                                     \
                    PS_WAIT_VM(63);                                                                                  \
            }                                                                                                        \
            else if (STAGES == 3 && u + 2 < ntrips)                                                                  \
                PS_WAIT_VM(DMA_PER_WAVE);                                                                            \
            else                                                                                                     \
                PS_WAIT_VM(0);                                                                                       \
        }                                                                                                            \
        PS_BARRIER()                                                                                                 \
        cur = cur + 1 == STAGES ? 0 : cur + 1;                                                                       \
        ++u;                                                                                                         \
    }
#define PS_C_FIRST_TAIL()                                                                                            \
    {                                                                                                                \
        PS_LOAD_KL(cur, 1)                                                                                           \
        PS_WAIT_LDS();                                                                                               \
        PS_STEP(1)                                                                                                   \
    }

    const int tab_trip = nk - 3;
    {
        if (issuer)
            PS_DMA_ISSUE(0)
        PS_DMA_ADVANCE()
        if (STAGES == 3)
        {
            if (issuer)
                PS_DMA_ISSUE(1)
            PS_DMA_ADVANCE()
            if (issuer)
                PS_WAIT_VM(DMA_PER_WAVE);
        }
        else if (issuer)
            PS_WAIT_VM(0);
    }
    PS_BARRIER()
    if (grp == 1)
        PS_BARRIER()
    PS_M(true, false, false, false, false, false)
    __builtin_amdgcn_s_setprio(1);
#pragma unroll
    for (int mi = 0; mi < MI; ++mi)
        PS_BAND(mi, 0, true)
    PS_C_FIRST_TAIL()
    __builtin_amdgcn_s_setprio(0);
    PS_C_END(false)
    [[maybe_unused]] long long pq_loop = 0, pq_epi = 0, pq_epi_m = 0, pq_t0 = 0, pq_t1 = 0, pq_t2 = 0;
    const long long pq_start = PS_PROFILE ? clock64() : 0;
    for (int tile = 0; tile < ntiles; ++tile)
    {
        if (PS_PROFILE)
            pq_t0 = clock64();
        for (int kt = 1; kt < nk; ++kt)
        {
            const bool tab = kt == tab_trip;
            PS_M(false, kt == 1, tile > 0 && kt == 1, tab, false, false)
            __builtin_amdgcn_s_setprio(1);
            PS_STEP(0)
            PS_STEP(1)
            __builtin_amdgcn_s_setprio(0);
            PS_C_END(tile > 0 && kt == 1 && STAGES == 3)
        }
        if (PS_PROFILE)
        {
            pq_t1 = clock64();
            pq_loop += pq_t1 - pq_t0;
        }
        e_m0 = c_m0;
        e_n0 = c_n0;
        e_tgi = c_tgi;
        e_ln0 = c_ln0;
        e_f0 = c_f0;
        if (tile + 1 < ntiles)
        {
            c_m0 = n_m0;
            c_n0 = n_n0;
            c_tgi = n_tgi;
            c_ln0 = n_ln0;
            c_f0 = n_f0;
            PS_M(true, false, false, false, true, true)
            if (PS_PROFILE)
            {
                pq_t2 = clock64();
                pq_epi_m += pq_t2 - pq_t1;
            }
            if (PS_PREWAIT && issuer)
                PS_WAIT_VM(0);
            PS_EPI_SETUP()
// ... 53 lines not shown
```

Measured before the change: 38910.

## Fuse FC1 fp16 plane split and row-sum partials into FC1 GEMM epilogue

The FC1 GEMM epilogue now writes its tanh outputs directly as two fp16 planes of the scaled value, plus per-64-column partial row sums, instead of writing f32 rows. The separate split_planes pass for the IH0 input is replaced by a small finish kernel that reduces the partials. This removes an f32 write and re-read of the FC1 activations and one kernel pass, at the cost of a heavier epilogue with DPP reductions and extra partial-sum storage. The f32 output is now written only when debug taps are enabled.

```diff
diff --git a/umx.cpp_amd/__init__.py b/umx.cpp_amd/__init__.py
--- a/umx.cpp_amd/__init__.py
+++ b/umx.cpp_amd/__init__.py
@@ -559,7 +559,7 @@
             return buf.reshape(2, T, NB)
         if what == "x":
             return buf.reshape(T, KX)
-        if what in ("fc1", "lstm", "fc2"):
+        if what in ("fc1", "lstm", "fc2", "fc1_plane1", "fc1_plane2"):
             return buf.reshape(T, H)
         if what == "mask":
             return buf.reshape(T, NOUT)
diff --git a/umx.cpp_amd/csrc/engine.hip b/umx.cpp_amd/csrc/engine.hip
--- a/umx.cpp_amd/csrc/engine.hip
+++ b/umx.cpp_amd/csrc/engine.hip
@@ -74,6 +74,7 @@
     unsigned short *xs_p = nullptr, *cat_p = nullptr, *la_p = nullptr, *lb_p = nullptr, *a2_p = nullptr;
     float *rs_xs = nullptr, *rs_catL = nullptr, *rs_catR = nullptr, *rs_la = nullptr, *rs_lb = nullptr, *rs_a2 = nullptr;
     float *rsc_xs = nullptr, *rsc_a2 = nullptr;
+    float *rs_catL_part = nullptr;
 };
 
 enum
@@ -154,6 +155,7 @@
     Lane lane[LSTMB_MAX_TRACKS];
     float *hbuf = nullptr;
     float *wv = nullptr;
+    bool fc1_rows_f32 = true;
     bool lstm_wrote_planes[3] = {false, false, false};
     bool lstm_rows_f32[3] = {true, true, true};
     unsigned *status = nullptr, *lsync = nullptr;
@@ -261,6 +263,9 @@
 
 #ifndef UMX_FUSE_LSTM_PLANES
 #define UMX_FUSE_LSTM_PLANES 1
+#endif
+#ifndef UMX_FUSE_FC1_PLANES
+#define UMX_FUSE_FC1_PLANES 1
 #endif
 enum { LSTM_PERSISTENT = 0, LSTM_BATCH, LSTM_BATCH8 };
 struct LstmKernel
@@ -466,6 +471,7 @@
     bool wiener_fused = true;
     bool gemm_planes = false;
     void launch_split(Lane &ln, int nl, hipStream_t st, int which, const int *active, int nact);
+    void launch_fc1_rowsums(Lane &ln, int nl, hipStream_t st, const int *active, int nact);
     void launch_gemm_planes(Lane &ln, int nl, hipStream_t st, int mode, int layer, const int *active, int nact, bool dbg);
     void launch_gemm_lanes(Slot &sl, hipStream_t st, int nb, const float *const *audio_dev, int mode, int layer, const int *active,
                            int nact, bool dbg);
@@ -481,6 +487,7 @@
     int env_lstm8_min = 1;
     bool lstm_rowsums = false;
     bool lstm_writes_planes = false;
+    bool fc1_writes_planes = false;
     size_t state_floats() const { return (size_t)4 * 12 * Hl; }
     int track(const float *audio_host, int length, int shift_offset, float *const out_host[4], unsigned flags,
               void (*progress)(float, void *), void *progress_user);
diff --git a/umx.cpp_amd/csrc/engine_cabi.h b/umx.cpp_amd/csrc/engine_cabi.h
--- a/umx.cpp_amd/csrc/engine_cabi.h
+++ b/umx.cpp_amd/csrc/engine_cabi.h
@@ -710,6 +710,28 @@
             return -1;
     }
     const Lane &sl = ctx->slot[which].lane[lane];
+    if (w == "fc1_plane1" || w == "fc1_plane2" || w == "fc1_rowsum")
+    {
+        const TargetAct &ta = sl.ta[target];
+        if (!ta.cat_p || !ta.rs_catL)
+            return -2;
+        const size_t n = w == "fc1_rowsum" ? (size_t)T : (size_t)T * H;
+        if (!dst)
+            return (long)n;
+        if (cap < n)
+            return -3;
+        if (ctx->sync_all() != UMX_OK)
+            return -4;
+        if (w == "fc1_rowsum")
+            return hipMemcpy(dst, ta.rs_catL, n * sizeof(float), hipMemcpyDeviceToHost) == hipSuccess ? (long)n : -4;
+        std::vector<unsigned short> bits(n);
+        const unsigned short *plane = ta.cat_p + (w == "fc1_plane2" ? ((size_t)ctx->B * ctx->Tp + ctx->Mpad) * 2 * H : 0);
+        if (hipMemcpy2D(bits.data(), (size_t)H * 2, plane, (size_t)2 * H * 2, (size_t)H * 2, T, hipMemcpyDeviceToHost) != hipSuccess)
+            return -4;
+        for (size_t i = 0; i < n; ++i)
+            dst[i] = f16_bits_to_float(bits[i]);
+        return (long)n;
+    }
     const void *src = nullptr;
     size_t nfl = 0, src_ld = 0, rows = 0, cols = 0;
     int computed = 0;
@@ -728,7 +750,7 @@
     else if (w == "max_abs") { src = sl.maxabs; nfl = 1; }
     else return -1;
     if ((w == "lstm" && !ctx->slot[which].lstm_rows_f32[2]) || (w == "lstm_l0" && !ctx->slot[which].lstm_rows_f32[0]) ||
-        (w == "lstm_l1" && !ctx->slot[which].lstm_rows_f32[1]))
+        (w == "lstm_l1" && !ctx->slot[which].lstm_rows_f32[1]) || (w == "fc1" && !ctx->slot[which].fc1_rows_f32))
         return -2;
     if (!src)
         return -2;
diff --git a/umx.cpp_amd/csrc/engine_init.h b/umx.cpp_amd/csrc/engine_init.h
--- a/umx.cpp_amd/csrc/engine_init.h
+++ b/umx.cpp_amd/csrc/engine_init.h
@@ -466,13 +466,16 @@
             if (int rc = dalloc(&mag_all, (size_t)B * 2 * T * MAGP))
                 return rc;
             unsigned short *xs_p = nullptr, *cat_p = nullptr, *la_p = nullptr, *lb_p = nullptr, *a2_p = nullptr;
-            float *rs[8] = {};
+            float *rs[8] = {}, *rs_part = nullptr;
             if (gemm_planes)
             {
                 if (int rc = dalloc(&xs_p, 2 * ((size_t)B * Tp + Mpad) * KX))
                     return rc;
-                if (int rc = dalloc(&cat_p, 2 * ((size_t)B * Tp + Mpad) * 2 * H))
+                const size_t cat_p_elems = 2 * ((size_t)B * Tp + Mpad) * 2 * H, part_elems = ((size_t)B * Tp + Mpad) * (H / 64);
+                if (int rc = dalloc(&cat_p, cat_p_elems + (UMX_FUSE_FC1_PLANES ? 2 * part_elems : 0)))
                     return rc;
+                if (UMX_FUSE_FC1_PLANES)
+                    rs_part = reinterpret_cast<float *>(cat_p + cat_p_elems);
                 for (unsigned short **q : {&la_p, &lb_p, &a2_p})
                     if (int rc = dalloc(q, 2 * ((size_t)B * Tp + Mpad) * H))
                         return rc;
@@ -504,6 +507,7 @@
                     b.rs_a2 = rs[5] + (size_t)ln * Tp;
                     b.rsc_xs = rs[6] + (size_t)ln * Tp;
                     b.rsc_a2 = rs[7] + (size_t)ln * Tp;
+                    b.rs_catL_part = rs_part ? rs_part + (size_t)ln * Tp : nullptr;
                 }
             }
         }
@@ -582,6 +586,7 @@
             lstm_batch_capacity = per_cu[lstm_batch8_ok ? LSTM_BATCH8 : LSTM_BATCH] * cus;
             lstm_rowsums = UMX_FUSE_LSTM_PLANES && gemm_planes && !u8_dequant && whh_q[0] && whh_q[1] && whh_q[2];
             lstm_writes_planes = lstm_rowsums;
+            fc1_writes_planes = UMX_FUSE_FC1_PLANES && lstm_rowsums;
         }
     }
     for (const void *fn : {reinterpret_cast<const void *>(wiener_istft_kernel<true>), reinterpret_cast<const void *>(wiener_istft_kernel<false>),
diff --git a/umx.cpp_amd/csrc/engine_stages.h b/umx.cpp_amd/csrc/engine_stages.h
--- a/umx.cpp_amd/csrc/engine_stages.h
+++ b/umx.cpp_amd/csrc/engine_stages.h
@@ -103,6 +103,24 @@
         hipLaunchKernelGGL(split_planes_kernel<6>, grid, dim3(256), 0, st, a);
     else
         hipLaunchKernelGGL(split_planes_kernel<8>, grid, dim3(256), 0, st, a);
+}
+
+void umx_hip_ctx::launch_fc1_rowsums(Lane &ln, int nl, hipStream_t st, const int *active, int nact)
+{
+    Fc1FinishArgs a;
+    memset(&a, 0, sizeof a);
+    for (int i = 0; i < nact; ++i)
+    {
+        a.part[i] = ln.ta[active[i]].rs_catL_part;
+        a.rowsum[i] = ln.ta[active[i]].rs_catL;
+    }
+    a.part_rows = (size_t)B * Tp + Mpad;
+    a.nparts = H / 64;
+    a.rows = round_up(nl * Tp, 256);
+    a.rows_valid = nl * Tp;
+    a.Tp = Tp;
+    a.T = T;
+    hipLaunchKernelGGL(fc1_rowsum_finish_kernel, dim3(a.rows / 256, nact), dim3(256), 0, st, a);
 }
 
 void umx_hip_ctx::launch_gemm_planes(Lane &ln, int nl, hipStream_t st, int mode, int layer, const int *active, int nact, bool dbg)
@@ -128,6 +146,12 @@
         {
         case G_FC1:
             t.A = c.xs_p; t.C = c.cat; t.rs0 = c.rs_xs; t.rsc = c.rsc_xs;
+            if (fc1_writes_planes)
+            {
+                t.Cp = c.cat_p; t.rs_part = c.rs_catL_part;
+                g.fc1_planes = 1; g.ldp = 2 * H; g.c_plane = rows_all * 2 * H; g.part_rows = rows_all;
+                g.write_f32 = dbg ? 1 : 0;
+            }
             t.e0 = b.bn1[0]; t.e1 = b.bn1[1]; t.e2 = b.bn1[2]; t.e3 = b.bn1[3];
             g.N = H; g.K = KX; g.lda = KX; g.ldc = 2 * H; g.a_plane = rows_all * KX;
             break;
@@ -196,7 +220,9 @@
         {
             const int which = mode == G_FC1 ? SP_XS : mode == G_IH ? (layer == 0 ? SP_CATL : layer == 1 ? SP_LA : SP_LB) : mode == G_FC2 ? SP_CATR : SP_A2;
             const int from_layer = which == SP_LA ? 0 : which == SP_LB ? 1 : which == SP_CATR ? 2 : -1;
-            if (from_layer < 0 || !sl.lstm_wrote_planes[from_layer])
+            if (which == SP_CATL && fc1_writes_planes)
+                launch_fc1_rowsums(sl.lane[l0], l1 - l0, st, active, nact);
+            else if (from_layer < 0 || !sl.lstm_wrote_planes[from_layer])
                 launch_split(sl.lane[l0], l1 - l0, st, which, active, nact);
             {
                 const int stg = mode == G_FC1 ? ST_FC1 : mode == G_IH ? ST_IH0 + 2 * layer : mode == G_FC2 ? ST_FC2 : ST_FC3;
@@ -232,7 +258,11 @@
     }
     stage_range(ST_FC1);
     UMX_HIP_CHECK(hipEventRecord(sl.ev[ST_FC1], st));
-    launch_gemm_lanes(sl, st, nb, audio_dev, G_FC1, 0, active, nact, false);
+    {
+        const bool taps = last_flags & UMX_FLAG_DEBUG_TAPS;
+        sl.fc1_rows_f32 = !(gemm_planes && fc1_writes_planes) || taps;
+        launch_gemm_lanes(sl, st, nb, audio_dev, G_FC1, 0, active, nact, taps);
+    }
     stage_range(ST_IH0);
     UMX_HIP_CHECK(hipEventRecord(sl.ev[ST_IH0], st));
     launch_gemm_lanes(sl, st, nb, audio_dev, G_IH, 0, active, nact, false);
diff --git a/umx.cpp_amd/csrc/gemm_common.h b/umx.cpp_amd/csrc/gemm_common.h
--- a/umx.cpp_amd/csrc/gemm_common.h
+++ b/umx.cpp_amd/csrc/gemm_common.h
@@ -154,6 +154,130 @@
     }
 }
 
+struct Fc1Planes
+{
+    unsigned short *P;
+    float *part;
+    size_t plane, part_rows;
+    int ldp, rows_valid, Tp, T, write_f32;
+};
+
+__device__ __forceinline__ unsigned fc1p_perm_sel(int lr) { return (lr & 1) ? 0x03020706u : 0x05040100u; }
+__device__ __forceinline__ int fc1p_col(int lr) { return (lr & 1) ? 31 + lr : lr; }
+__device__ __forceinline__ void fc1_plane_words(float v0, float v1, unsigned sel, unsigned &w1, unsigned &w2)
+{
+    typedef _Float16 f16x2 __attribute__((ext_vector_type(2)));
+    const float s0 = v0 * (float)(1 << 14), s1 = v1 * (float)(1 << 14);
+    f16x2 h1, h2;
+    h1[0] = (_Float16)s0;
+    h1[1] = (_Float16)s1;
+    h2[0] = (_Float16)(s0 - (float)h1[0]);
+    h2[1] = (_Float16)(s1 - (float)h1[1]);
+    const unsigned p1 = __builtin_bit_cast(unsigned, h1), p2 = __builtin_bit_cast(unsigned, h2);
+    const unsigned x1 = (unsigned)__builtin_amdgcn_update_dpp(0, (int)p1, 0xB1, 0xf, 0xf, true);
+    const unsigned x2 = (unsigned)__builtin_amdgcn_update_dpp(0, (int)p2, 0xB1, 0xf, 0xf, true);
+    w1 = __builtin_amdgcn_perm(x1, p1, sel);
+    w2 = __builtin_amdgcn_perm(x2, p2, sel);
+}
+template <int CTRL, int ROW_MASK> __device__ __forceinline__ float fc1p_dpp_add(float s)
+{
+    return s + __int_as_float(__builtin_amdgcn_update_dpp(0, __float_as_int(s), CTRL, ROW_MASK, 0xf, ROW_MASK == 0xf));
+}
+__device__ __forceinline__ float fc1_rowsum64(float v0, float v1)
+{
+    float s = v0 + v1;
+    s = fc1p_dpp_add<0xB1, 0xf>(s);
+    s = fc1p_dpp_add<0x4E, 0xf>(s);
+    s = fc1p_dpp_add<0x141, 0xf>(s);
+    s = fc1p_dpp_add<0x140, 0xf>(s);
+    return fc1p_dpp_add<0x142, 0xa>(s);
+}
+__device__ __forceinline__ float fc1p_pick(const float (&s)[4], int lr)
+{
+    const int j = lr & 3;
+    return j == 0 ? s[0] : j == 1 ? s[1] : j == 2 ? s[2] : s[3];
+}
+
+__device__ __forceinline__ void gemm_epilogue_fc1_planes(const GemmTarget &tg, const GemmArgs &args, const Fc1Planes &fp, int m0, int n0, int wn, int lr,
+                                                         int lh, const floatx16 &acc00, const floatx16 &acc01, const floatx16 &acc10,
+                                                         const floatx16 &acc11)
+{
+    float rm[2], sd[2], rsd[2], gw[2], gb[2];
+#pragma unroll
+    for (int ni = 0; ni < 2; ++ni)
+    {
+        const int n = n0 + wn * 64 + ni * 32 + lr;
+        rm[ni] = tg.e0[n];
+        sd[ni] = sqrtf(tg.e1[n] + 1e-5f);
+        rsd[ni] = 1.0f / sd[ni];
+        gw[ni] = tg.e2[n];
+        gb[ni] = tg.e3[n];
+    }
+    const unsigned sel = fc1p_perm_sel(lr);
+    const int nb = n0 + wn * 64;
+    const int f0 = m0 - __builtin_amdgcn_readfirstlane(m0 / fp.Tp) * fp.Tp;
+    float *const part = fp.part + (size_t)(nb >> 6) * fp.part_rows;
+#pragma unroll
+    for (int mi = 0; mi < 2; ++mi)
+#pragma unroll
+        for (int rq = 0; rq < 4; ++rq)
+        {
+            float s[4];
+#pragma unroll
+            for (int j = 0; j < 4; ++j)
+            {
+                const int r = 4 * rq + j;
+                const int ml = mi * 32 + j + 8 * rq + 4 * lh;
+                float y0 = mi == 0 ? acc00[r] : acc10[r], y1 = mi == 0 ? acc01[r] : acc11[r];
+                y0 = tanh_epi(div_by(y0 - rm[0], sd[0], rsd[0]) * gw[0] + gb[0]);
+                y1 = tanh_epi(div_by(y1 - rm[1], sd[1], rsd[1]) * gw[1] + gb[1]);
+                unsigned w1, w2;
+                fc1_plane_words(y0, y1, sel, w1, w2);
+                s[j] = fc1_rowsum64(y0, y1);
+                const int m = m0 + ml, f1 = f0 + ml, f = f1 >= fp.Tp ? f1 - fp.Tp : f1;
+                if (m < fp.rows_valid && f < fp.T)
+                {
+                    unsigned *const p = reinterpret_cast<unsigned *>(fp.P + (size_t)m * fp.ldp + nb) + (fc1p_col(lr) >> 1);
+                    __builtin_nontemporal_store(w1, p);
+                    __builtin_nontemporal_store(w2, p + (fp.plane >> 1));
+                }
+                if (fp.write_f32)
+                {
+                    tg.C[(size_t)m * args.ldc + nb + lr] = y0;
+                    tg.C[(size_t)m * args.ldc + nb + 32 + lr] = y1;
+                }
+            }
+            const float sv = fc1p_pick(s, lr);
+            if (lr >= 16 && lr < 20)
+                part[m0 + mi * 32 + 8 * rq + 4 * lh + (lr & 3)] = sv;
+            asm volatile("" ::: "memory");
+            __builtin_amdgcn_sched_barrier(0);
+        }
+}
+
+struct Fc1FinishArgs
+{
+    const float *part[4];
+    float *rowsum[4];
+    size_t part_rows;
+    int nparts, rows, rows_valid, Tp, T;
+};
+__global__ __launch_bounds__(256) void fc1_rowsum_finish_kernel(Fc1FinishArgs a)
+{
+    const int m = blockIdx.x * 256 + threadIdx.x, tg = blockIdx.y;
+    if (m >= a.rows)
+        return;
+    float s = 0.f;
+    if (m < a.rows_valid && m % a.Tp < a.T)
+    {
+        const float *p = a.part[tg] + m;
+        s = p[0];
+        for (int b = 1; b < a.nparts; ++b)
+            s += p[(size_t)b * a.part_rows];
+    }
+    a.rowsum[tg][m] = s;
+}
+
 enum GemmBType
 {
     BQ_F32 = 0,
diff --git a/umx.cpp_amd/csrc/gemm_planes.h b/umx.cpp_amd/csrc/gemm_planes.h
--- a/umx.cpp_amd/csrc/gemm_planes.h
+++ b/umx.cpp_amd/csrc/gemm_planes.h
@@ -16,6 +16,8 @@
     const float *rsc;
     float bs[2], bo2[2];
     int bsplit;
+    unsigned short *Cp;
+    float *rs_part;
 };
 
 struct GemmPArgs
@@ -27,7 +29,24 @@
     int Tp_lane;
     int lanes;
     size_t mag_lane;
+    int fc1_planes, write_f32, ldp;
+    size_t c_plane, part_rows;
 };
+
+__device__ __forceinline__ Fc1Planes fc1_planes_of(const GemmPTarget &tg, const GemmPArgs &args)
+{
+    Fc1Planes fp;
+    fp.P = tg.Cp;
+    fp.part = tg.rs_part;
+    fp.plane = args.c_plane;
+    fp.part_rows = args.part_rows;
+    fp.ldp = args.ldp;
+    fp.rows_valid = args.lanes * args.Tp_lane;
+    fp.Tp = args.Tp_lane;
+    fp.T = args.T;
+    fp.write_f32 = args.write_f32;
+    return fp;
+}
 
 constexpr int GP_BK = 32;
 constexpr int GP_SPLIT_FIXED_EXP = 14;
@@ -481,6 +500,15 @@
     ea.Tp_lane = args.Tp_lane;
     ea.lanes = args.lanes;
     ea.mag_lane = args.mag_lane;
+    if (MODE == G_FC1 && args.fc1_planes)
+    {
+        const Fc1Planes fp = fc1_planes_of(tg, args);
+#pragma unroll
+        for (int half = 0; half < MI / 2; ++half)
+            gemm_epilogue_fc1_planes(et, ea, fp, m0 + wm * 32 * MI + half * 64, n0, wn, lr, lh, acc[2 * half][0], acc[2 * half][1],
+                                     acc[2 * half + 1][0], acc[2 * half + 1][1]);
+        return;
+    }
 #pragma unroll
     for (int half = 0; half < MI / 2; ++half)
         gemm_epilogue<MODE>(et, ea, m0 + wm * 32 * MI + half * 64, n0, 0, wn, lr, lh, acc[2 * half][0], acc[2 * half][1], acc[2 * half + 1][0],
diff --git a/umx.cpp_amd/csrc/gemm_planes_pp.h b/umx.cpp_amd/csrc/gemm_planes_pp.h
--- a/umx.cpp_amd/csrc/gemm_planes_pp.h
+++ b/umx.cpp_amd/csrc/gemm_planes_pp.h
@@ -248,10 +248,21 @@
             tg.C[tid] = s;
         return;
     }
-#pragma unroll
-    for (int half = 0; half < MI / 2; ++half)
-        gemm_epilogue<MODE>(et, ea, m0 + wm * 32 * MI + half * 64, n0, 0, wn, lr, lh, acc[2 * half][0], acc[2 * half][1], acc[2 * half + 1][0],
-                            acc[2 * half + 1][1]);
+    if (MODE == G_FC1 && args.fc1_planes)
+    {
+        const Fc1Planes fp = fc1_planes_of(tg, args);
+#pragma unroll
+        for (int half = 0; half < MI / 2; ++half)
+            gemm_epilogue_fc1_planes(et, ea, fp, m0 + wm * 32 * MI + half * 64, n0, wn, lr, lh, acc[2 * half][0], acc[2 * half][1],
+                                     acc[2 * half + 1][0], acc[2 * half + 1][1]);
+    }
+    else
+    {
+#pragma unroll
+        for (int half = 0; half < MI / 2; ++half)
+            gemm_epilogue<MODE>(et, ea, m0 + wm * 32 * MI + half * 64, n0, 0, wn, lr, lh, acc[2 * half][0], acc[2 * half][1], acc[2 * half + 1][0],
+                                acc[2 * half + 1][1]);
+    }
     if (PP_PROFILE)
     {
         pq[4] = clock64();
diff --git a/umx.cpp_amd/csrc/gemm_planes_ps.h b/umx.cpp_amd/csrc/gemm_planes_ps.h
--- a/umx.cpp_amd/csrc/gemm_planes_ps.h
+++ b/umx.cpp_amd/csrc/gemm_planes_ps.h
@@ -54,7 +54,7 @@
         TGI = tg_;                                                                                                   \
         M0 = (first_m_ + in_group_ - q_ * gsize_) * BM;                                                              \
         N0 = q_ * BN;                                                                                                \
-        if (MODE == G_FC3)                                                                                           \
+        if (MODE == G_FC3 || MODE == G_FC1)             \
         {                                                                                                            \
             LN0 = M0 / args.Tp_lane;                                                                                 \
             F0 = M0 - LN0 * args.Tp_lane;                                                                            \
@@ -183,6 +183,9 @@
     float4 nx_mu, nx_ad;
     uint4 nx_ro;
     int e_row = 0;
+    const bool fc1p = MODE == G_FC1 && args.fc1_planes;
+    unsigned pco = 0, psel = 0, rso = 0, so_p2 = 0, so_rs = 0;
+    int pj = 0;
 #define PS_EPI_ROWS(g_)                                                                                              \
     {                                                                                                                \
         nx_mu = row4[e_row + 2 * (g_)];                                                                              \
@@ -213,6 +216,17 @@
                 cvo[ni] = reinterpret_cast<const unsigned *>(coltab)[7 * 256 + cl_];                                 \
             }                                                                                                        \
         }                                                                                                            \
+        if (fc1p)                                                                                                    \
+        {                                                                                                            \
+            const int lr_ = el_ & 31;                                                                                \
+            pj = lr_ & 3;                                                                                            \
+            psel = fc1p_perm_sel(lr_);                                                                               \
+            pco = (unsigned)(wn * 128 + fc1p_col(lr_) * 2);                                                          \
+            rso = lr_ >= 16 && lr_ < 20 ? (unsigned)(pj + 4 * (el_ >> 5)) * 4u : PS_DROP;                            \
+            unsigned char *const p1_ = reinterpret_cast<unsigned char *>(args.t[e_tgi].Cp) + ((size_t)e_m0 * args.ldp + e_n0) * 2; \
+            so_p2 = (unsigned)(args.c_plane * 2);                                                                    \
+            so_rs = (unsigned)(reinterpret_cast<unsigned char *>(args.t[e_tgi].rs_part + ((size_t)((e_n0 >> 6) + wn) * args.part_rows + e_m0)) - p1_); \
+        }                                                                                                            \
         PS_EPI_ROWS(0)                                                                                               \
         if (MODE == G_FC3)                                                                                           \
         {                                                                                                            \
@@ -221,6 +235,8 @@
             rsC = __builtin_amdgcn_make_buffer_rsrc(reinterpret_cast<unsigned char *>(args.t[e_tgi].C) + lo_, 0,     \
                                                     (int)(rest_ < 2 * lane_b_ ? rest_ : 2 * lane_b_), 0x00020000);   \
         }                                                                                                            \
+        else if (fc1p)                                                                                               \
+            rsC = __builtin_amdgcn_make_buffer_rsrc(args.t[e_tgi].Cp + ((size_t)e_m0 * args.ldp + e_n0), 0, 256 * args.ldp * 2, 0x00020000); \
         else                                                                                                         \
             rsC = __builtin_amdgcn_make_buffer_rsrc(args.t[e_tgi].C + ((size_t)e_m0 * args.ldc + e_n0), 0, 0x7fffffff, 0x00020000); \
     }
@@ -252,10 +268,40 @@
                 ys_[ni][j] = y;                                                                                      \
                 os_[ni][j] = ro_[j] + cvo[ni];                                                                       \
             }                                                                                                        \
-        __builtin_amdgcn_sched_barrier(0);  \
-        _Pragma("unroll") for (int ni = 0; ni < 2; ++ni)                                                             \
+        if (fc1p)                                                                                                    \
+        {                                                                                                            \
+             \
+            unsigned w1_[4], w2_[4];                                                                                 \
+            float s_[4];                                                                                             \
             _Pragma("unroll") for (int j = 0; j < 4; ++j)                                                            \
-                __builtin_amdgcn_raw_buffer_store_b32(__float_as_uint(ys_[ni][j]), rsC, os_[ni][j], 0, PS_STORE_AUX);   \
+            {                                                                                                        \
+                fc1_plane_words(ys_[0][j], ys_[1][j], psel, w1_[j], w2_[j]);                                         \
+                s_[j] = fc1_rowsum64(ys_[0][j], ys_[1][j]);                                                          \
+            }                                                                                                        \
+            const float sv_ = pj == 0 ? s_[0] : pj == 1 ? s_[1] : pj == 2 ? s_[2] : s_[3];                           \
+            __builtin_amdgcn_sched_barrier(0);                                                                       \
+            _Pragma("unroll") for (int j = 0; j < 4; ++j)                                                            \
+            {                                                                                                        \
+                __builtin_amdgcn_raw_buffer_store_b32(w1_[j], rsC, ro_[j] + pco, 0, PS_STORE_AUX);                   \
+                __builtin_amdgcn_raw_buffer_store_b32(w2_[j], rsC, ro_[j] + pco, so_p2, PS_STORE_AUX);               \
+            }                                                                                                        \
+            __builtin_amdgcn_raw_buffer_store_b32(__float_as_uint(sv_), rsC, rso + (unsigned)(((mi)*32 + 8 * rq) * 4), so_rs, 0); \
+            if (args.write_f32)  \
+            {                                                                                                        \
+                const __amdgpu_buffer_rsrc_t rsF_ =                                                                  \
+                    __builtin_amdgcn_make_buffer_rsrc(args.t[e_tgi].C + ((size_t)e_m0 * args.ldc + e_n0), 0, 0x7fffffff, 0x00020000); \
+                _Pragma("unroll") for (int ni = 0; ni < 2; ++ni)                                                     \
+                    _Pragma("unroll") for (int j = 0; j < 4; ++j)                                                    \
+                        __builtin_amdgcn_raw_buffer_store_b32(__float_as_uint(ys_[ni][j]), rsF_, 2u * ro_[j] + cvo[ni], 0, PS_STORE_AUX); \
+            }                                                                                                        \
+        }                                                                                                            \
+        else                                                                                                         \
+        {                                                                                                            \
+            __builtin_amdgcn_sched_barrier(0);  \
+            _Pragma("unroll") for (int ni = 0; ni < 2; ++ni)                                                         \
+                _Pragma("unroll") for (int j = 0; j < 4; ++j)                                                        \
+                    __builtin_amdgcn_raw_buffer_store_b32(__float_as_uint(ys_[ni][j]), rsC, os_[ni][j], 0, PS_STORE_AUX); \
+        }                                                                                                            \
         __builtin_amdgcn_sched_barrier(0);                                                                           \
     }
 
@@ -308,6 +354,12 @@
                                                       \
                 const int f1_ = e_f0 + tid, second_ = f1_ >= args.Tp_lane ? 1 : 0, f_ = f1_ - second_ * args.Tp_lane; \
                 off_ = f_ < args.T ? ((unsigned)second_ * (unsigned)args.mag_lane + (unsigned)f_ * MAGP) * 4u : PS_DROP; \
+            }                                                                                                        \
+            if (fc1p)                                                                                                \
+            {                                                                                                        \
+                 \
+                const int f1_ = e_f0 + tid, f_ = f1_ >= args.Tp_lane ? f1_ - args.Tp_lane : f1_;                     \
+                off_ = f_ < args.T && e_m0 + tid < args.lanes * args.Tp_lane ? (unsigned)tid * (unsigned)args.ldp * 2u : PS_DROP; \
             }                                                                                                        \
             rowtab[tid] = tg_.bs[sel_] * rsc_;                            \
             rowtab[256 + tid] = tg_.bo2[sel_] * (tg_.rs2 ? (r0_ + r1_) + r2_ : tg_.rs1 ? r0_ + r1_ : r0_);           \
```

Result: no change. 39010, median of 3 (+0.3%).
